# Cjen1/stateright

Measured on AMD Instinct MI355X. Metric: unique states/sec (whole node) + HBM GB/s, 2pc N=9 at 1/2/4/8 MI355X, higher is better.
Workload: dtype u64; 1 GPU; 2pc N=9 spawn_bfs, full check per step (10340352 unique states); model=2pc, rm_count=9, order=fast, parallelism=1 GPU, world_size=1

## Files before the change

include/stateright_gpu.h:

```cpp
#ifndef STATERIGHT_GPU_H
#define STATERIGHT_GPU_H

#include <stdint.h>

#ifdef __cplusplus
extern "C" {
#endif

enum sr_model_id {
    SR_MODEL_LINEAR_EQUATION = 1,
    SR_MODEL_BINARY_CLOCK = 2,
    SR_MODEL_2PC = 3,
    SR_MODEL_INCREMENT = 4,
    SR_MODEL_INCREMENT_LOCK = 5,
    SR_MODEL_DGRAPH = 6,
    SR_MODEL_PAXOS = 7,
    SR_MODEL_PINGPONG = 9,
    SR_MODEL_ACTOR_FIXTURE = 10,
    SR_MODEL_ABD = 11,
    SR_MODEL_SINGLE_COPY = 12,
    SR_MODEL_LADDER = 13,
    SR_MODEL_SPREAD = 14
};

enum sr_order {
    SR_ORDER_AUTO = 0,
    SR_ORDER_FIFO = 1,
    SR_ORDER_FAST = 2
};

enum sr_expectation { SR_ALWAYS = 0, SR_EVENTUALLY = 1, SR_SOMETIMES = 2 };

enum sr_status {
    SR_OK = 0,
    SR_ERR_ARG = -1,
    SR_ERR_HIP = -2,
    SR_ERR_CAPACITY = -3,
    SR_ERR_UNSUPPORTED = -4,
    SR_ERR_NO_DEVICE = -5,
    SR_ERR_NONDETERMINISM = -6
};

typedef struct sr_opts {
    uint32_t struct_size;
    int32_t device;
    uint64_t target_state_count;
    int32_t order;
    int32_t record_visits;
    uint64_t capacity_hint;
    int32_t profile;
    int32_t verbose;
    int32_t counters;
    int32_t defer_paths;
    int32_t symmetry;
} sr_opts;

typedef struct sr_stats {
    double level_loop_sec;
    double total_sec;
    double expand_kernel_ms;
    uint64_t expand_launches;
    uint64_t levels;
    uint64_t table_capacity;
    uint64_t rehashes;
    uint64_t algorithmic_bytes;
    uint64_t successors;
    uint32_t words_per_state;
    uint32_t order_used;
    uint32_t restarts;
    uint32_t pipelined;
    uint64_t records_routed;
    uint64_t head_levels;
    uint64_t probes;
    uint64_t cas;
    uint64_t max_displacement;
    uint32_t displacement_limit;
    uint32_t table_doublings;
    uint32_t exchange_fallbacks;
    uint32_t owner_key;
    uint32_t balanced_levels;
    uint32_t table_encoding;
} sr_stats;

typedef struct sr_bfs sr_bfs;

void sr_opts_init(sr_opts* opts);
void sr_opts_init_sized(sr_opts* opts, uint32_t size);
const char* sr_last_error(void);
int sr_device_count(void);

sr_bfs* sr_gpu_bfs_spawn(int32_t model_id, const int64_t* params, int32_t nparams, const sr_opts* opts);
int32_t sr_gpu_bfs_join(sr_bfs* bfs);
int32_t sr_gpu_bfs_is_done(const sr_bfs* bfs);
int32_t sr_gpu_bfs_is_running(const sr_bfs* bfs);
uint64_t sr_gpu_bfs_state_count(const sr_bfs* bfs);
uint64_t sr_gpu_bfs_unique_state_count(const sr_bfs* bfs);
uint32_t sr_gpu_bfs_max_depth(const sr_bfs* bfs);
int32_t sr_gpu_bfs_stats(const sr_bfs* bfs, sr_stats* out);
int32_t sr_gpu_bfs_stats_sized(const sr_bfs* bfs, sr_stats* out, uint32_t size);
int64_t sr_gpu_bfs_launch_profile(const sr_bfs* bfs, double* kernel_ms, uint64_t* frontier, int64_t cap);
int64_t sr_gpu_bfs_launch_counters(const sr_bfs* bfs, uint64_t* probes, uint64_t* cas, int64_t cap);

int32_t sr_gpu_bfs_property_count(const sr_bfs* bfs);
int32_t sr_gpu_bfs_property(const sr_bfs* bfs, int32_t prop, char* name, int32_t cap, int32_t* expectation);

int32_t sr_gpu_bfs_discovery(const sr_bfs* bfs, int32_t prop, uint64_t* fp_chain, uint32_t cap);
int32_t sr_gpu_bfs_discovery_path(const sr_bfs* bfs, int32_t prop, int64_t* action_ids, int32_t cap_actions,
                                  int64_t* states, int64_t cap_states);
int32_t sr_gpu_bfs_describe_width(const sr_bfs* bfs);
int32_t sr_gpu_bfs_action_name(const sr_bfs* bfs, int64_t action_id, char* buf, int32_t cap);
int64_t sr_gpu_bfs_action_id_bound(const sr_bfs* bfs);
int32_t sr_gpu_bfs_init_count(const sr_bfs* bfs);
int32_t sr_gpu_bfs_replay(const sr_bfs* bfs, int32_t init_index, const int64_t* action_ids, int32_t n_actions,
                          int64_t* states, int64_t cap_states, int32_t* conditions, int32_t cap_conditions);
int32_t sr_gpu_bfs_replay_trace(const sr_bfs* bfs, int32_t init_index, const int64_t* action_ids, int32_t n_actions,
                                int32_t* conditions, int64_t cap, int32_t* terminal);
int32_t sr_gpu_bfs_explore(const sr_bfs* bfs, const uint64_t* fingerprints, int32_t n, int64_t* action_ids,
                           int32_t* has_state, uint64_t* fingerprints_out, int64_t* states, int32_t cap);
int64_t sr_gpu_bfs_visits(const sr_bfs* bfs, int64_t* out, int64_t cap);
int64_t sr_gpu_bfs_visit_tree(const sr_bfs* bfs, int64_t* parent, int64_t* action, int64_t cap);
void sr_gpu_bfs_free(sr_bfs* bfs);

#define SR_DIST_ID_BYTES 128
typedef struct sr_dist sr_dist;
int32_t sr_dist_unique_id(uint8_t* id_out);
sr_dist* sr_dist_init(int32_t rank, int32_t world, const uint8_t* id, int32_t device);
int32_t sr_dist_local_group(int32_t world, const int32_t* devices, sr_dist** comms_out);
sr_dist* sr_dist_shm_init(int32_t rank, int32_t world, const char* name, int32_t device, int64_t slot_bytes,
                          int32_t devices_distinct);
int32_t sr_dist_rank(const sr_dist* comm);
int32_t sr_dist_world(const sr_dist* comm);
int32_t sr_dist_nranks(const sr_dist* comm);
int32_t sr_dist_kind(const sr_dist* comm, char* buf, int32_t cap);
int32_t sr_dist_barrier(sr_dist* comm);
int32_t sr_dist_allreduce_f64(sr_dist* comm, double* values, int32_t n, int32_t op);
void sr_dist_free(sr_dist* comm);

typedef struct sr_dist_host_opts {
    uint32_t struct_size;
    int32_t rm_count;
    uint64_t cmin;
    int32_t corrupt_level;
    int32_t capacity_fail_at_end;
    int32_t fail_at_end;
    int32_t plan_div;
} sr_dist_host_opts;
typedef struct sr_dist_host_result {
    uint64_t unique, state_count, local_unique;
    uint32_t max_depth, levels;
    uint32_t attempts, restarts, fallbacks, disagreements;
    uint32_t overflow_level;
    uint32_t first_outcome;
    uint64_t plan_digest;
} sr_dist_host_result;
int32_t sr_dist_host_protocol(const char* name, int32_t rank, int32_t world, const sr_dist_host_opts* opts,
                              sr_dist_host_result* out);

int32_t sr_rccl_version(int32_t* runtime, int32_t* compiled);
int32_t sr_hip_runtime_version(int32_t* runtime, int32_t* compiled);
int32_t sr_device_synchronize(int32_t device);
const char* sr_build_digest(void);
int32_t sr_selftest_tables(void);
int32_t sr_selftest_level_geometry(void);
int32_t sr_selftest_models(void);
int32_t sr_selftest_action_masks(void);
int32_t sr_selftest_table_growth(void);
int32_t sr_table_encoding(int32_t words, int32_t key_bits, uint64_t slots, uint32_t* out);
sr_bfs* sr_gpu_bfs_spawn_partitioned(sr_dist* comm, int32_t virtual_partitions, int32_t model_id,
                                     const int64_t* params, int32_t nparams, const sr_opts* opts);

#define SR_PLUGIN_ABI 4
typedef struct sr_plugin {
    uint32_t abi;
    uint32_t opts_size;
    const char* name;
    void* (*create)(const int64_t* params, int32_t nparams, const sr_opts* opts, void* comm, int32_t virtual_parts,
                    char* err, int32_t errcap);
    int32_t (*fingerprint)(const int64_t* params, int32_t nparams, const int64_t* described, int32_t width,
                           uint64_t* fp_out);
} sr_plugin;

sr_bfs* sr_gpu_bfs_spawn_plugin(const sr_plugin* plugin, const int64_t* params, int32_t nparams, const sr_opts* opts);
sr_bfs* sr_gpu_bfs_spawn_plugin_partitioned(const sr_plugin* plugin, sr_dist* comm, int32_t virtual_partitions,
                                            const int64_t* params, int32_t nparams, const sr_opts* opts);

int32_t sr_model_fingerprint(int32_t model_id, const int64_t* params, int32_t nparams, const int64_t* described,
                             int32_t width, uint64_t* fp_out);
int64_t sr_selftest_describe(int32_t model_id, const int64_t* params, int32_t nparams, int64_t max_states);

#ifdef __cplusplus
}
#endif
#endif
```

stateright_amd/_native.py:

```python
import ctypes
import os

HERE = os.path.dirname(os.path.abspath(__file__))
LIB_PATH = os.environ.get("SR_LIB_PATH") or os.path.join(HERE, "libstateright_gpu.so")

SR_MODEL_LINEAR_EQUATION = 1
SR_MODEL_BINARY_CLOCK = 2
SR_MODEL_2PC = 3
SR_MODEL_INCREMENT = 4
SR_MODEL_INCREMENT_LOCK = 5
SR_MODEL_DGRAPH = 6
SR_MODEL_PAXOS = 7
SR_MODEL_PINGPONG = 9
SR_MODEL_ACTOR_FIXTURE = 10
SR_MODEL_ABD = 11
SR_MODEL_SINGLE_COPY = 12
SR_MODEL_LADDER = 13
SR_MODEL_SPREAD = 14

SR_ORDER_AUTO, SR_ORDER_FIFO, SR_ORDER_FAST = 0, 1, 2
SR_ALWAYS, SR_EVENTUALLY, SR_SOMETIMES = 0, 1, 2


class sr_opts(ctypes.Structure):
    _fields_ = [
        ("struct_size", ctypes.c_uint32),
        ("device", ctypes.c_int32),
        ("target_state_count", ctypes.c_uint64),
        ("order", ctypes.c_int32),
        ("record_visits", ctypes.c_int32),
        ("capacity_hint", ctypes.c_uint64),
        ("profile", ctypes.c_int32),
        ("verbose", ctypes.c_int32),
        ("counters", ctypes.c_int32),
        ("defer_paths", ctypes.c_int32),
        ("symmetry", ctypes.c_int32),
    ]


class sr_stats(ctypes.Structure):
    _fields_ = [
        ("level_loop_sec", ctypes.c_double),
        ("total_sec", ctypes.c_double),
        ("expand_kernel_ms", ctypes.c_double),
        ("expand_launches", ctypes.c_uint64),
        ("levels", ctypes.c_uint64),
        ("table_capacity", ctypes.c_uint64),
        ("rehashes", ctypes.c_uint64),
        ("algorithmic_bytes", ctypes.c_uint64),
        ("successors", ctypes.c_uint64),
        ("words_per_state", ctypes.c_uint32),
        ("order_used", ctypes.c_uint32),
        ("restarts", ctypes.c_uint32),
        ("pipelined", ctypes.c_uint32),
        ("records_routed", ctypes.c_uint64),
        ("head_levels", ctypes.c_uint64),
        ("probes", ctypes.c_uint64),
        ("cas", ctypes.c_uint64),
        ("max_displacement", ctypes.c_uint64),
        ("displacement_limit", ctypes.c_uint32),
        ("table_doublings", ctypes.c_uint32),
        ("exchange_fallbacks", ctypes.c_uint32),
        ("owner_key", ctypes.c_uint32),
        ("balanced_levels", ctypes.c_uint32),
        ("table_encoding", ctypes.c_uint32),
    ]

    def as_dict(self):
        return {name: getattr(self, name) for name, _ in self._fields_}


class sr_dist_host_opts(ctypes.Structure):
    _fields_ = [
        ("struct_size", ctypes.c_uint32),
        ("rm_count", ctypes.c_int32),
        ("cmin", ctypes.c_uint64),
        ("corrupt_level", ctypes.c_int32),
        ("capacity_fail_at_end", ctypes.c_int32),
        ("fail_at_end", ctypes.c_int32),
        ("plan_div", ctypes.c_int32),
    ]


class sr_dist_host_result(ctypes.Structure):
    _fields_ = [
        ("unique", ctypes.c_uint64),
        ("state_count", ctypes.c_uint64),
        ("local_unique", ctypes.c_uint64),
        ("max_depth", ctypes.c_uint32),
        ("levels", ctypes.c_uint32),
        ("attempts", ctypes.c_uint32),
        ("restarts", ctypes.c_uint32),
        ("fallbacks", ctypes.c_uint32),
        ("disagreements", ctypes.c_uint32),
        ("overflow_level", ctypes.c_uint32),
        ("first_outcome", ctypes.c_uint32),
        ("plan_digest", ctypes.c_uint64),
    ]

    def as_dict(self):
        return {name: getattr(self, name) for name, _ in self._fields_}


_P = ctypes.c_void_p
_I64P = ctypes.POINTER(ctypes.c_int64)
SIGNATURES = [
    ("sr_opts_init", None, [ctypes.POINTER(sr_opts)]),
    ("sr_opts_init_sized", None, [ctypes.POINTER(sr_opts), ctypes.c_uint32]),
    ("sr_last_error", ctypes.c_char_p, []),
    ("sr_device_count", ctypes.c_int, []),
    ("sr_gpu_bfs_spawn", _P, [ctypes.c_int32, _I64P, ctypes.c_int32, ctypes.POINTER(sr_opts)]),
    ("sr_gpu_bfs_join", ctypes.c_int32, [_P]),
    ("sr_gpu_bfs_is_done", ctypes.c_int32, [_P]),
    ("sr_gpu_bfs_is_running", ctypes.c_int32, [_P]),
    ("sr_gpu_bfs_state_count", ctypes.c_uint64, [_P]),
    ("sr_gpu_bfs_unique_state_count", ctypes.c_uint64, [_P]),
    ("sr_gpu_bfs_max_depth", ctypes.c_uint32, [_P]),
    ("sr_gpu_bfs_stats", ctypes.c_int32, [_P, ctypes.POINTER(sr_stats)]),
    ("sr_gpu_bfs_stats_sized", ctypes.c_int32, [_P, ctypes.POINTER(sr_stats), ctypes.c_uint32]),
    ("sr_gpu_bfs_launch_counters", ctypes.c_int64, [_P, ctypes.POINTER(ctypes.c_uint64), ctypes.POINTER(ctypes.c_uint64),
                                                    ctypes.c_int64]),
    ("sr_gpu_bfs_launch_profile", ctypes.c_int64, [_P, ctypes.POINTER(ctypes.c_double), ctypes.POINTER(ctypes.c_uint64),
                                                   ctypes.c_int64]),
    ("sr_gpu_bfs_property_count", ctypes.c_int32, [_P]),
    ("sr_gpu_bfs_property", ctypes.c_int32, [_P, ctypes.c_int32, ctypes.c_char_p, ctypes.c_int32,
                                             ctypes.POINTER(ctypes.c_int32)]),
    ("sr_gpu_bfs_discovery", ctypes.c_int32, [_P, ctypes.c_int32, ctypes.POINTER(ctypes.c_uint64), ctypes.c_uint32]),
    ("sr_gpu_bfs_discovery_path", ctypes.c_int32, [_P, ctypes.c_int32, _I64P, ctypes.c_int32, _I64P, ctypes.c_int64]),
    ("sr_gpu_bfs_describe_width", ctypes.c_int32, [_P]),
    ("sr_gpu_bfs_action_name", ctypes.c_int32, [_P, ctypes.c_int64, ctypes.c_char_p, ctypes.c_int32]),
    ("sr_gpu_bfs_action_id_bound", ctypes.c_int64, [_P]),
    ("sr_gpu_bfs_init_count", ctypes.c_int32, [_P]),
    ("sr_gpu_bfs_replay", ctypes.c_int32, [_P, ctypes.c_int32, _I64P, ctypes.c_int32, _I64P, ctypes.c_int64,
                                           ctypes.POINTER(ctypes.c_int32), ctypes.c_int32]),
    ("sr_gpu_bfs_replay_trace", ctypes.c_int32, [_P, ctypes.c_int32, _I64P, ctypes.c_int32, ctypes.POINTER(ctypes.c_int32),
                                                 ctypes.c_int64, ctypes.POINTER(ctypes.c_int32)]),
    ("sr_gpu_bfs_explore", ctypes.c_int32, [_P, ctypes.POINTER(ctypes.c_uint64), ctypes.c_int32, _I64P,
                                            ctypes.POINTER(ctypes.c_int32), ctypes.POINTER(ctypes.c_uint64), _I64P,
                                            ctypes.c_int32]),
    ("sr_gpu_bfs_visits", ctypes.c_int64, [_P, _I64P, ctypes.c_int64]),
    ("sr_gpu_bfs_visit_tree", ctypes.c_int64, [_P, _I64P, _I64P, ctypes.c_int64]),
    ("sr_gpu_bfs_free", None, [_P]),
    ("sr_dist_unique_id", ctypes.c_int32, [ctypes.c_char_p]),
    ("sr_dist_init", _P, [ctypes.c_int32, ctypes.c_int32, ctypes.c_char_p, ctypes.c_int32]),
    ("sr_dist_local_group", ctypes.c_int32, [ctypes.c_int32, ctypes.POINTER(ctypes.c_int32), ctypes.POINTER(_P)]),
    ("sr_dist_shm_init", _P, [ctypes.c_int32, ctypes.c_int32, ctypes.c_char_p, ctypes.c_int32, ctypes.c_int64,
                              ctypes.c_int32]),
    ("sr_dist_rank", ctypes.c_int32, [_P]),
    ("sr_dist_world", ctypes.c_int32, [_P]),
    ("sr_dist_nranks", ctypes.c_int32, [_P]),
    ("sr_dist_kind", ctypes.c_int32, [_P, ctypes.c_char_p, ctypes.c_int32]),
    ("sr_dist_barrier", ctypes.c_int32, [_P]),
    ("sr_dist_allreduce_f64", ctypes.c_int32, [_P, ctypes.POINTER(ctypes.c_double), ctypes.c_int32, ctypes.c_int32]),
    ("sr_dist_free", None, [_P]),
    ("sr_dist_host_protocol", ctypes.c_int32, [ctypes.c_char_p, ctypes.c_int32, ctypes.c_int32,
                                               ctypes.POINTER(sr_dist_host_opts), ctypes.POINTER(sr_dist_host_result)]),
    ("sr_rccl_version", ctypes.c_int32, [ctypes.POINTER(ctypes.c_int32), ctypes.POINTER(ctypes.c_int32)]),
    ("sr_hip_runtime_version", ctypes.c_int32, [ctypes.POINTER(ctypes.c_int32), ctypes.POINTER(ctypes.c_int32)]),
    ("sr_device_synchronize", ctypes.c_int32, [ctypes.c_int32]),
    ("sr_build_digest", ctypes.c_char_p, []),
    ("sr_selftest_tables", ctypes.c_int32, []),
    ("sr_selftest_level_geometry", ctypes.c_int32, []),
    ("sr_selftest_models", ctypes.c_int32, []),
    ("sr_selftest_action_masks", ctypes.c_int32, []),
    ("sr_selftest_table_growth", ctypes.c_int32, []),
    ("sr_table_encoding", ctypes.c_int32, [ctypes.c_int32, ctypes.c_int32, ctypes.c_uint64, ctypes.POINTER(ctypes.c_uint32)]),
    ("sr_gpu_bfs_spawn_plugin", _P, [_P, _I64P, ctypes.c_int32, ctypes.POINTER(sr_opts)]),
    ("sr_gpu_bfs_spawn_plugin_partitioned", _P, [_P, _P, ctypes.c_int32, _I64P, ctypes.c_int32,
                                                 ctypes.POINTER(sr_opts)]),
    ("sr_model_fingerprint", ctypes.c_int32, [ctypes.c_int32, _I64P, ctypes.c_int32, _I64P, ctypes.c_int32,
                                              ctypes.POINTER(ctypes.c_uint64)]),
    ("sr_selftest_describe", ctypes.c_int64, [ctypes.c_int32, _I64P, ctypes.c_int32, ctypes.c_int64]),
    ("sr_gpu_bfs_spawn_partitioned", _P, [_P, ctypes.c_int32, ctypes.c_int32, _I64P, ctypes.c_int32,
                                          ctypes.POINTER(sr_opts)]),
]

SR_DIST_ID_BYTES = 128

_lib = None


def load():
    global _lib
    if _lib is None:
        if not os.path.exists(LIB_PATH):
            raise ImportError(
                f"MI355X engine library not found at {LIB_PATH}; build it with "
                "`python -c 'import __graft_entry__ as g; g.build()'` (hipcc --offload-arch=gfx950)")
        lib = ctypes.CDLL(LIB_PATH)
        ab = os.environ.get("SR_LIB_DIGEST_CHECK", "1") == "0"
        for name, res, args in SIGNATURES:
            fn = getattr(lib, name, None)
            if fn is None and ab:
                continue
            if fn is None:
                raise ImportError(f"{LIB_PATH} lacks {name}: rebuild it")
            fn.restype = res
            fn.argtypes = args
        check_digest(lib)
        _lib = lib
    return _lib


class StaleLibraryError(ImportError):
    pass


def check_digest(lib, sources_root=None):
    if os.environ.get("SR_LIB_DIGEST_CHECK", "1") == "0":
        return
    from . import build
    want = build.source_digest() if sources_root is None else build.source_digest_at(sources_root)
    got = lib.sr_build_digest().decode()
    if got != want:
        raise StaleLibraryError(
            f"{LIB_PATH} was built from sources with digest {got}, but the sources here have digest {want}; "
            "rebuild it (`python -c 'import __graft_entry__ as g; g.build()'`)")


def build_digest():
    lib = load()
    return lib.sr_build_digest().decode() if hasattr(lib, "sr_build_digest") else "unstamped"


def last_error():
    return load().sr_last_error().decode(errors="replace")


def table_encoding(words, key_bits, slots):
    out = (ctypes.c_uint32 * 8)()
    st = load().sr_table_encoding(words, key_bits, slots, out)
    if st != 0:
        raise ValueError(f"sr_table_encoding: {last_error()} (status {st})")
    return dict(zip(("qbits", "dbits", "bbits", "plimit", "s32", "filter", "filter_log2", "min_cap_log2"), out))


def runtime_versions():
    lib = load()
    out = {}
    for key, fn in (("hip", lib.sr_hip_runtime_version), ("rccl", lib.sr_rccl_version)):
        r, c = ctypes.c_int32(), ctypes.c_int32()
        out[key] = (r.value, c.value) if fn(ctypes.byref(r), ctypes.byref(c)) == 0 else (None, None)
    return out


def loaded_runtime_paths():
    paths = set()
    try:
        with open("/proc/self/maps") as f:
            for line in f:
                p = line.split()[-1] if line.count(" ") >= 5 else ""
                if "libamdhip64" in p or "librccl" in p:
                    paths.add(p)
    except OSError:
        pass
    return sorted(paths)
```

stateright_amd/csrc/device.hpp:

```cpp
#pragma once
#include <hip/hip_runtime.h>

#include <chrono>
#include <cstdint>
#include <cstdio>
#include <cstdlib>
#include <cstring>
#include <map>
#include <mutex>
#include <stdexcept>
#include <string>
#include <tuple>
#include <vector>

namespace sr {

struct Error : std::runtime_error {
    int code;
    Error(int c, const std::string& m) : std::runtime_error(m), code(c) {}
};

#define SR_HIP(expr)                                                                              \
    do {                                                                                          \
        hipError_t e_ = (expr);                                                                   \
        if (e_ != hipSuccess)                                                                     \
            throw ::sr::Error(-2, std::string(#expr) + ": " + hipGetErrorString(e_) + " at " +   \
                                      __FILE__ + ":" + std::to_string(__LINE__));                 \
    } while (0)

inline void clear_not_ready() {
    if (hipPeekAtLastError() == hipErrorNotReady) (void)hipGetLastError();
}
inline hipError_t stream_sync(hipStream_t s) {
    const auto t0 = std::chrono::steady_clock::now();
    for (unsigned spin = 1;; ++spin) {
        const hipError_t e = hipStreamQuery(s);
        if (e != hipErrorNotReady) {
            if (spin > 1) clear_not_ready();
            return e;
        }
        if ((spin & 255) == 0 && std::chrono::steady_clock::now() - t0 > std::chrono::microseconds(500))
            return clear_not_ready(), hipStreamSynchronize(s);
        __builtin_ia32_pause();
    }
}

struct StreamCensus {
    static StreamCensus& get() {
        static StreamCensus c;
        return c;
    }
    void created(int dev) {
        std::lock_guard<std::mutex> g(mu_);
        ++n_[dev];
    }
    void destroyed(int dev) {
        std::lock_guard<std::mutex> g(mu_);
        --n_[dev];
    }
    int on(int dev) {
        std::lock_guard<std::mutex> g(mu_);
        return n_[dev];
    }
    static int hw_queues() {
        const char* e = std::getenv("GPU_MAX_HW_QUEUES");
        return e && std::atoi(e) > 0 ? std::atoi(e) : 4;
    }
    std::mutex mu_;
    std::map<int, int> n_;
};
inline hipError_t create_stream(hipStream_t* s, int dev) {
    const hipError_t e = hipStreamCreateWithFlags(s, hipStreamNonBlocking);
    if (e == hipSuccess) StreamCensus::get().created(dev);
    return e;
}

class DevicePool {
  public:
    static DevicePool& get() {
        static DevicePool p;
        return p;
    }
    void* alloc(int dev, size_t bytes, int kind = 0) {
        bytes = round(bytes);
        {
            std::lock_guard<std::mutex> g(mu_);
            auto& fl = free_[{dev, bytes, kind}];
            if (!fl.empty()) {
                void* p = fl.back();
                fl.pop_back();
                return p;
            }
            if (kind == 0)
                if (void* p = take_zeroed_locked(dev, bytes)) return p;
        }
        void* p = nullptr;
        auto raw = [&]() {
            return kind == 1   ? hipExtMallocWithFlags(&p, bytes, hipDeviceMallocFinegrained)
                   : kind == 2 ? hipExtMallocWithFlags(&p, bytes, hipDeviceMallocUncached)
                               : hipMalloc(&p, bytes);
        };
        const auto t0 = std::chrono::steady_clock::now();
        hipError_t e = raw();
        const bool retried = e != hipSuccess;
        if (retried) {
            release_all(dev);
            (void)hipGetLastError();
            SR_HIP(raw());
        }
        if (trace())
            std::fprintf(stderr, "[pool] device %d: %zu bytes (kind %d) fresh%s in %.3f ms\n", dev, bytes, kind,
                         retried ? " after emptying the cache" : "",
                         std::chrono::duration<double, std::milli>(std::chrono::steady_clock::now() - t0).count());
        return p;
    }
    void free(int dev, void* p, size_t bytes, int kind = 0) {
        if (!p) return;
        std::lock_guard<std::mutex> g(mu_);
        free_[{dev, round(bytes), kind}].push_back(p);
    }
    void free_zeroed(int dev, void* p, size_t bytes, hipEvent_t ready, int kind = 0) {
        std::lock_guard<std::mutex> g(mu_);
        zeroed_[{dev, round(bytes), kind}].push_back({p, ready});
    }
    void* alloc_zeroed(int dev, size_t bytes, hipStream_t s, int kind = 0) {
        Zeroed z{nullptr, nullptr};
        {
            std::lock_guard<std::mutex> g(mu_);
            auto& fl = zeroed_[{dev, round(bytes), kind}];
            if (fl.empty()) return nullptr;
            size_t pick = 0;
            for (size_t i = 0; i < fl.size(); ++i)
                if (hipEventQuery(fl[i].ready) == hipSuccess) {
                    pick = i;
                    break;
                }
            clear_not_ready();
            z = fl[pick];
            fl.erase(fl.begin() + (long)pick);
        }
        const hipError_t e = hipStreamWaitEvent(s, z.ready, 0);
        if (e != hipSuccess) {
            (void)hipEventSynchronize(z.ready);
            (void)hipEventDestroy(z.ready);
            free(dev, z.p, bytes, kind);
            return nullptr;
        }
        (void)hipEventDestroy(z.ready);
        return z.p;
    }
    void release_all(int dev) {
        std::lock_guard<std::mutex> g(mu_);
        ++epoch_[dev];
        for (auto& [k, v] : free_)
            if (std::get<0>(k) == dev) {
                for (void* p : v) (void)hipFree(p);
                v.clear();
            }
        for (auto& [k, v] : zeroed_)
            if (std::get<0>(k) == dev) {
                for (auto& z : v) {
                    (void)hipEventSynchronize(z.ready);
                    (void)hipEventDestroy(z.ready);
                    (void)hipFree(z.p);
                }
                v.clear();
            }
    }
    static bool trace() {
        static const bool on = std::getenv("SR_POOL_TRACE") && std::atoi(std::getenv("SR_POOL_TRACE")) != 0;
        return on;
    }
    static size_t round(size_t b) {
        if (b < 256) return 256;
        if (b >= (2u << 20)) return (b + (2u << 20) - 1) & ~(size_t)((2u << 20) - 1);
        size_t r = 256;
        while (r < b) r <<= 1;
        return r;
    }

    uint64_t epoch(int dev) {
        std::lock_guard<std::mutex> g(mu_);
        return epoch_[dev];
    }

  private:
    struct Zeroed {
        void* p;
        hipEvent_t ready;
    };
    void* take_zeroed_locked(int dev, size_t bytes) {
        auto it = zeroed_.find({dev, bytes, 0});
        if (it == zeroed_.end()) return nullptr;
        auto& fl = it->second;
        for (size_t i = 0; i < fl.size(); ++i) {
            if (hipEventQuery(fl[i].ready) != hipSuccess) continue;
            Zeroed z = fl[i];
            fl.erase(fl.begin() + (long)i);
            (void)hipEventDestroy(z.ready);
            clear_not_ready();
            return z.p;
        }
        clear_not_ready();
        return nullptr;
    }
    std::mutex mu_;
    std::map<std::tuple<int, size_t, int>, std::vector<void*>> free_;
    std::map<std::tuple<int, size_t, int>, std::vector<Zeroed>> zeroed_;
    std::map<int, uint64_t> epoch_;
};

template <class T>
struct DBuf {
    T* p = nullptr;
    size_t n = 0;
    int dev = 0;
    int kind = 0;
    DBuf() = default;
    DBuf(const DBuf&) = delete;
    DBuf& operator=(const DBuf&) = delete;
    DBuf(DBuf&& o) noexcept { swap(o); }
    ~DBuf() { reset(); }
    void reset() {
        if (p) DevicePool::get().free(dev, p, n * sizeof(T), kind);
        p = nullptr;
        n = 0;
        kind = 0;
    }
    void alloc(int d, size_t count, int k = 0) {
        reset();
        dev = d;
        n = count ? count : 1;
        kind = k;
        p = static_cast<T*>(DevicePool::get().alloc(d, n * sizeof(T), k));
    }
    void alloc_zero(int d, size_t count, hipStream_t s, int k = 0) {
        reset();
        dev = d;
        n = count ? count : 1;
        kind = k;
        p = static_cast<T*>(DevicePool::get().alloc_zeroed(d, n * sizeof(T), s, k));
        if (p) return;
        p = static_cast<T*>(DevicePool::get().alloc(d, n * sizeof(T), k));
        SR_HIP(hipMemsetAsync(p, 0, n * sizeof(T), s));
    }
    void release_zero(hipStream_t s) noexcept {
        if (!p) return;
        hipEvent_t ready = nullptr;
        if (hipEventCreateWithFlags(&ready, hipEventDisableTiming) == hipSuccess) {
            if (hipMemsetAsync(p, 0, n * sizeof(T), s) == hipSuccess && hipEventRecord(ready, s) == hipSuccess) {
                DevicePool::get().free_zeroed(dev, p, n * sizeof(T), ready, kind);
                p = nullptr;
                n = 0;
                kind = 0;
                return;
            }
            (void)hipEventDestroy(ready);
        }
        (void)hipStreamSynchronize(s);
        (void)hipGetLastError();
        reset();
    }
    void swap(DBuf& o) {
        std::swap(p, o.p);
        std::swap(n, o.n);
        std::swap(dev, o.dev);
        std::swap(kind, o.kind);
    }
};

template <class Counters, class HostMirror>
struct DeviceContext {
    int dev = 0;
    hipStream_t stream = nullptr;
    Counters* lc = nullptr;
    HostMirror* hc = nullptr;
    HostMirror* hc_dev = nullptr;
    uint32_t seq = 0;
    std::vector<hipEvent_t> events;
    hipEvent_t done = nullptr;

    void init(int d) {
        dev = d;
        SR_HIP(hipSetDevice(d));
        SR_HIP(create_stream(&stream, d));
        SR_HIP(hipEventCreateWithFlags(&done, hipEventDisableTiming));
        SR_HIP(hipMalloc(&lc, sizeof(Counters)));
        SR_HIP(hipHostMalloc(&hc, 2 * sizeof(HostMirror), hipHostMallocCoherent | hipHostMallocMapped));
        SR_HIP(hipHostGetDevicePointer(reinterpret_cast<void**>(&hc_dev), hc, 0));
        std::memset(hc, 0, 2 * sizeof(HostMirror));
    }
    hipEvent_t event(size_t i) {
        while (events.size() <= i) {
            hipEvent_t e;
            SR_HIP(hipEventCreate(&e));
            events.push_back(e);
        }
        return events[i];
    }
};

template <class Ctx>
class ContextPool {
  public:
    static ContextPool& get() {
        static ContextPool p;
        return p;
    }
    Ctx* acquire(int dev) {
        {
            std::lock_guard<std::mutex> g(mu_);
            auto& fl = free_[dev];
            if (!fl.empty()) {
                Ctx* c = fl.back();
                fl.pop_back();
                return c;
            }
        }
        auto* c = new Ctx();
        c->init(dev);
        return c;
    }
    void release(Ctx* c) {
        if (!c) return;
        std::lock_guard<std::mutex> g(mu_);
        free_[c->dev].push_back(c);
    }

  private:
    std::mutex mu_;
    std::map<int, std::vector<Ctx*>> free_;
};

}
// ... 1 lines not shown
```

stateright_amd/csrc/engine.hip:

```cpp
#include <unordered_set>
#include "registry.hpp"
#include "dgraph.hpp"
#include "paxos.hpp"
#include "abd_wide.hpp"
#include "dist_host.hpp"
#include "table_selftest.hpp"

namespace sr {

static thread_local std::string g_last_error;
static void set_error(const std::string& e) { g_last_error = e; }

}

namespace sr {

static std::unique_ptr<EngineBase> make_model_engine(const EngineArgs& a) {
    if (a.o->symmetry && a.model != SR_MODEL_2PC)
        throw Error(SR_ERR_UNSUPPORTED, "symmetry reduction: model " + std::to_string(a.model) + " has no canonical form");
    switch (a.model) {
        case SR_MODEL_LINEAR_EQUATION:
        case SR_MODEL_BINARY_CLOCK:
        case SR_MODEL_DGRAPH:
        case SR_MODEL_ACTOR_FIXTURE:
// ... 812 lines not shown
int32_t sr_hip_runtime_version(int32_t* runtime, int32_t* compiled) {
    int v = 0;
    if (hipRuntimeGetVersion(&v) != hipSuccess) return SR_ERR_HIP;
    if (runtime) *runtime = v;
    if (compiled) *compiled = HIP_VERSION;
    return SR_OK;
}

int32_t sr_selftest_tables(void) {
    for (u32 B = 1; B <= 18; ++B) {
        std::vector<u8> seen(1u << B, 0);
        for (u64 x = 0; x < (1ull << B); ++x) {
            const u64 y = (u64)qperm(x, B);
            if (y >> B || seen[y]) {
                set_error("qperm is not a bijection on " + std::to_string(B) + " bits");
                return SR_ERR_ARG;
            }
            seen[y] = 1;
        }
    }
    for (u32 B = 2; B <= 20; ++B) {
        std::vector<u8> seen(1u << B, 0);
        for (u64 x = 0; x < (1ull << B); ++x) {
            const u64 y = qmix(x, B);
            if (y >> B || seen[y]) {
                set_error("qmix is not a bijection on " + std::to_string(B) + " bits");
                return SR_ERR_ARG;
            }
            seen[y] = 1;
        }
    }
    const u32 ncases[][2] = {{40, 25}, {40, 22}, {44, 27}, {48, 29}, {52, 31}, {16, 22}, {62, 40}};
    u64 rn = 0x452821E638D01377ull;
    for (auto& c : ncases) {
        const u32 q = c[0] > c[1] ? c[0] - c[1] : 1u;
        TableView t{nullptr, nullptr, (1ull << c[1]) - 1, q, 32 - q, c[0]};
        t.s32 = 1;
        if (q + SLOT32_DMIN > 32) {
            t.s32 = 0;
            t.dbits = 64 - q;
        }
        for (int i = 0; i < 100000; ++i) {
            rn = fmix64(rn + 0x9E3779B97F4A7C15ull);
            const u64 key = rn & ((1ull << c[0]) - 1);
            const u64 h = qmix(key, c[0]);
            const ProbeKey pk = quot_probe(t, h);
            const u64 d = (rn >> 40) % 500;
            const u64 slotv = pk.tag + d;
            if ((t.s32 && slotv >> 32) || quot_decode(t, (pk.home + d) & t.mask, slotv) != h || pk.home > t.mask ||
                filter_key(t, pk) != h + 1) {
                set_error("narrow quotient slot encode/decode mismatch at B=" + std::to_string(c[0]));
                return SR_ERR_ARG;
            }
        }
    }
    const u32 cases[][2] = {{89, 33}, {68, 20}, {82, 26}, {120, 64}};
    u64 r = 0x243F6A8885A308D3ull;
    for (auto& c : cases) {
        TableView t{nullptr, nullptr, (c[1] >= 64 ? ~0ull : (1ull << c[1]) - 1), c[0] - c[1], 64 - (c[0] - c[1]), c[0]};
        for (int i = 0; i < 100000; ++i) {
            r = fmix64(r + 0x9E3779B97F4A7C15ull);
            const u64 r2 = fmix64(r ^ 0xABCDEFull);
            const u128 key = ((u128)r2 << 64 | r) & (((u128)1 << c[0]) - 1);
            const u128 h = qperm(key, c[0]);
            const ProbeKey pk = quot_probe(t, h);
            const u64 d = r2 % 200;
            if (quot_decode(t, (pk.home + d) & t.mask, pk.tag + d) != h || pk.home > t.mask || (pk.tag & ((1ull << t.dbits) - 1)) != 1) {
                set_error("quotient slot encode/decode mismatch at B=" + std::to_string(c[0]));
                return SR_ERR_ARG;
            }
        }
    }
    return SR_OK;
}

int32_t sr_selftest_table_growth(void) {
    try {
        std::string why;
        if (!table_growth_selftest(why)) {
            set_error(why);
            return SR_ERR_ARG;
        }
        return SR_OK;
    } catch (const std::exception& x) {
        set_error(x.what());
        return SR_ERR_ARG;
    }
}

int32_t sr_table_encoding(int32_t words, int32_t key_bits, uint64_t slots, uint32_t* out) {
    try {
        if (!out || key_bits < 2 || (words != 1 && words != 2 && words != 4) || key_bits > std::min(64 * words, 128) ||
            !slots || (slots & (slots - 1)))
            throw Error(SR_ERR_ARG, "sr_table_encoding: words 1, 2 or 4, 2 <= key_bits <= min(64 words, 128), slots a power of two");
        const TableEncoding e = words == 1   ? table_encoding_of<1>(key_bits, slots)
                                : words == 2 ? table_encoding_of<2>(key_bits, slots)
                                             : table_encoding_of<4>(key_bits, slots);
        const u32 v[8] = {e.qbits, e.dbits, e.bbits, e.plimit, e.s32, e.filter, e.filter_log2, e.min_cap_log2};
        std::copy(v, v + 8, out);
        return SR_OK;
    } catch (const Error& x) {
        set_error(x.what());
        return x.code;
    } catch (const std::exception& x) {
        set_error(x.what());
        return SR_ERR_ARG;
    }
}

static bool check_level_geometry(u32 nblk, std::vector<u32>& stamp, std::vector<u32>& end, u32& gen,
                                 const std::vector<u32>& ns, std::string& why) {
    for (u32 wpb : {4u, 8u})
        for (u32 cap_log2 = 2; cap_log2 <= 6; ++cap_log2)
            for (int balanced = 0; balanced < 2; ++balanced)
                for (u32 n : ns) {
                    const u32 cap = 1u << cap_log2, lo = n & 1 ? 77u : 0u, hi = lo + n;
                    const LevelGeom g = level_geometry(n, nblk, wpb, cap, balanced != 0);
                    auto fail = [&](const char* what) {
                        why = std::string("level geometry: ") + what + " at n=" + std::to_string(n) + " nblk=" +
                              std::to_string(nblk) + " cap=" + std::to_string(cap) + " wpb=" + std::to_string(wpb) +
                              (balanced ? " balanced" : " fixed");
                        return false;
                    };
                    if (g.pw == 0 || g.pw > cap || g.cw == 0 || g.cw > wpb * cap) return fail("pw or cw out of range");
                    if (!balanced && (g.pw != cap || g.cw != wpb * cap)) return fail("fixed geometry changed");
                    ++gen;
                    u64 intervals = 0, share_min = ~0ull, share_max = 0;
                    for (u32 b = 0; b < nblk; ++b) {
                        u64 share = 0;
                        u64 j = 0;
                        for (u64 c0 = g.first_chunk(lo, b); c0 < hi; c0 += g.stride(nblk), ++j) {
                            const u32 lim = g.chunk_end(c0, hi);
                            for (u32 wid = 0; wid < wpb; ++wid) {
                                const u64 w0 = g.wave_first(c0, wid);
                                const u64 w1 = std::min<u64>(w0 + g.pw, lim);
                                if (!balanced) {
                                    const u64 o0 = lo + (((u64)b + j * nblk) * wpb << cap_log2) + ((u64)wid << cap_log2);
                                    const u64 o1 = std::min<u64>(o0 + cap, hi);
                                    if (o0 < o1 ? o0 != w0 || o1 != w1 : w0 < w1) return fail("differs from the shift formula");
                                }
                                if (w1 <= w0) continue;
                                if (w0 < lo || w1 > hi) return fail("a parent outside the frontier");
                                if (stamp[w0 - lo] == gen) return fail("a parent taken twice");
                                stamp[w0 - lo] = gen;
                                end[w0 - lo] = (u32)(w1 - lo);
                                share += w1 - w0;
                                ++intervals;
                            }
                        }
                        share_min = std::min(share_min, share);
                        share_max = std::max(share_max, share);
                    }
                    u64 followed = 0;
                    u32 pos = 0;
                    while (pos < n) {
                        if (stamp[pos] != gen) return fail("a parent not taken");
                        pos = end[pos];
                        ++followed;
                    }
                    if (pos != n || followed != intervals) return fail("waves overlap");
                    if (share_max - share_min > g.cw) return fail("workgroup shares differ by more than one chunk");
                }
    return true;
}

int32_t sr_selftest_level_geometry(void) {
// ... 167 lines not shown
```

stateright_amd/csrc/engine.hpp:

```cpp
#pragma once
#include <algorithm>
#include <atomic>
#include <chrono>
#include <cmath>
#include <cstdio>
#include <cstdlib>
#include <cstring>
#include <deque>
#include <immintrin.h>
#include <memory>
#include <string>
#include <thread>
#include <vector>

#include "../../include/stateright_gpu.h"
#include "device.hpp"
#include "kernels.hpp"

namespace sr {


using Clock = std::chrono::steady_clock;
static double secs(Clock::time_point a, Clock::time_point b) { return std::chrono::duration<double>(b - a).count(); }

// ... 179 lines not shown
        cur.clear();
        for (int i = 0; i < k && cur.empty(); ++i) {
            u64 c[W];
            m.base().canonical(&inits[i * W], c);
            if (std::equal(c, c + W, st.begin())) cur.assign(&inits[i * W], &inits[i * W] + W);
        }
        if (cur.empty()) throw Error(SR_ERR_NONDETERMINISM, "Unable to reconstruct a `Path`: no init state has the expected representative");
    }
    auto emit = [&](const u64* s) {
        const size_t o = states.size();
        states.resize(o + wd);
        m.describe(s, &states[o]);
        if (raw) raw->insert(raw->end(), s, s + W);
    };
    for (size_t i = 1; i < len; ++i) {
        const u64* target = &st[i * W];
        u64 mask[M::MW];
        m.enabled(cur.data(), mask);
        bool found = false;
        for (int w = 0; w < M::MW && !found; ++w)
            for (u64 bits = mask[w]; bits && !found; bits &= bits - 1) {
                const int a = w * 64 + __builtin_ctzll(bits);
                u64 ns[W];
                if (!m.apply(cur.data(), a, ns) || !std::equal(ns, ns + W, target)) continue;
                u64 next[W];
                if constexpr (is_canon<M>::value) m.base().apply(cur.data(), a, next);
                else std::copy(ns, ns + W, next);
                emit(cur.data());
                actions.push_back(m.action_id(cur.data(), a));
                cur.assign(next, next + W);
                found = true;
            }
        if (!found)
            throw Error(SR_ERR_NONDETERMINISM, "Unable to reconstruct a `Path`: " + std::to_string(i) +
                                                   " previous state(s) reconstructed but no successor is the next state");
    }
    emit(cur.data());
    return (int)actions.size();
}

template <class M>
int fingerprint_chain(const M& m, const std::vector<u64>& st, std::vector<u64>& out) {
    constexpr int W = M::W;
    out.clear();
    std::vector<u64> raw;
    if constexpr (is_canon<M>::value) {
        std::vector<i64> actions, described;
        concrete_path(m, st, actions, described, &raw);
    } else {
        raw = st;
    }
    for (size_t i = 0; i < raw.size() / W; ++i) out.push_back(state_fp<M>(&raw[i * W]));
    return (int)out.size();
}

template <class M>
class Engine final : public EngineBase {
    static constexpr int W = M::W;
    static constexpr u32 WPB = (u32)expand_wpb<M>();

  public:
    Engine(M m, const sr_opts& o)
        : m_(m), o_(o), A_((u32)m.max_actions()), D_((u32)m.max_out_degree()), emask_(model_emask(m)) {
        disc.resize(M::NPROPS);
        (void)init_states_of(m_);
        if (const char* e = std::getenv("SR_PROBE_BATCH")) probe_batch_ = std::atoi(e);
        if (const char* e = std::getenv("SR_TABLE_LOAD")) table_load_ = std::atof(e), load_env_ = true;
        if (const char* e = std::getenv("SR_PPW_LOG2")) ppw_env_ = std::atoi(e);
        if (const char* e = std::getenv("SR_FILTER_LOG2")) filt_log2_ = (u32)std::atoi(e);
        if (!filter_exact(m_)) filt_log2_ = 0;
        if (filt_log2_ && (!std::getenv("SR_FILTER_COMPACT") || std::atoi(std::getenv("SR_FILTER_COMPACT"))) &&
            filter_compact_ok(m_, filt_log2_ + 1))
            filt_log2_ += 1, filt_compact_ = true;
        grid_res_ = W == 1 ? 1u : 2u;
        if (const char* e = std::getenv("SR_GRID_RES"))
            if (std::atoi(e) > 0) grid_res_ = (u32)std::atoi(e);
        if (const char* e = std::getenv("SR_PIPELINE")) pipeline_ = std::atoi(e) != 0;
        if (const char* e = std::getenv("SR_QUERY_LOG2")) query_mask_ = (1ull << std::atoi(e)) - 1;
        if (const char* e = std::getenv("SR_GRID_MAX")) grid_env_ = (u32)std::max(0, std::atoi(e));
        if (const char* e = std::getenv("SR_WIDE_NOPF")) wide_nopf_ = std::atoi(e) ? 1 : 0;
        if (const char* e = std::getenv("SR_CHAIN_MAX")) chain_max_ = (u64)std::max(0ll, std::atoll(e));
        if (const char* e = std::getenv("SR_TABLE_KIND")) table_kind_ = std::atoi(e);
        if (const char* e = std::getenv("SR_TABLE_RECYCLE")) table_recycle_ = std::atoi(e) != 0;
        if (const char* e = std::getenv("SR_BALANCE")) balance_ = std::atoi(e) != 0;
        if (const char* e = std::getenv("SR_BALANCE_MIN")) balance_min_ = (u64)std::max(0ll, std::atoll(e));
        action_table_ = action_table_model<M> && A_ <= 64;
        if (const char* e = std::getenv("SR_ACTION_TABLE")) action_table_ = action_table_ && std::atoi(e) != 0;
    }
    ~Engine() override = default;

    int nprops() const override { return M::NPROPS; }
    const char* prop_name(int p) const override { return m_.prop_name(p); }
    int expectation(int p) const override { return m_.expectation(p); }
    int width() const override { return m_.describe_width(); }
    std::string action_name(i64 id) const override { return m_.action_name(id); }

    void run() override {
        SR_HIP(hipSetDevice(o_.device));
        CtxLease lease(o_.device);
        bind(lease.c);
        int order = o_.order;
        if (order == SR_ORDER_AUTO) order = o_.target_state_count ? SR_ORDER_FIFO : SR_ORDER_FAST;
        if (emask_ && o_.order != SR_ORDER_FAST) order = SR_ORDER_FIFO;
        bool order_dependent = run_with_restart(order);
        if (order_dependent && o_.order == SR_ORDER_AUTO && order == SR_ORDER_FAST) {
            if (o_.verbose) std::fprintf(stderr, "[sr] early exit in FAST order; re-running in FIFO order\n");
            run_with_restart(SR_ORDER_FIFO);
        }
        bind(nullptr);
    }

    bool run_with_restart(int order) {
        for (int attempt = 0;; ++attempt) {
            try {
                return run_order(order);
            } catch (const Error& e) {
                if (e.code != SR_ERR_CAPACITY || attempt >= 3) throw;
                if (o_.verbose) std::fprintf(stderr, "[sr] %s; restarting with larger buffers\n", e.what());
                pessimistic_ = true;
                grow_factor_ *= 4;
                (void)stream_sync(stream_);
                rehash_pending_ = false;
                retired_keys_.clear();
                retired_arena_.clear();
                retired_u32_.clear();
                init_counters();
            }
        }
    }

    int chain(int p, std::vector<u64>& out) override {
        out.clear();
        if (p < 0 || p >= M::NPROPS || !disc[p].found) return 0;
        SR_HIP(hipSetDevice(o_.device));
        std::vector<u64> st;
        tree_path(disc[p].level, disc[p].rank, st);
        return fingerprint_chain(m_, st, out);
    }

    void tree_path(u32 level, u32 rank, std::vector<u64>& st) {
        std::vector<u64> idx;
        u64 r = rank;
        for (int d = (int)level;; --d) {
            u64 a = lstart_[d] + r;
            idx.push_back(a);
            if (d == 0) break;
            u32 pr = 0;
            SR_HIP(hipMemcpy(&pr, apar_.p + a, sizeof(u32), hipMemcpyDeviceToHost));
            r = pr;
        }
        std::reverse(idx.begin(), idx.end());
        st.resize(idx.size() * W);
        for (size_t i = 0; i < idx.size(); ++i)
            SR_HIP(hipMemcpy(&st[i * W], arena_.p + idx[i] * W, W * sizeof(u64), hipMemcpyDeviceToHost));
    }

    int path(int p, std::vector<i64>& actions, std::vector<i64>& states) override {
        if (p < 0 || p >= M::NPROPS || !disc[p].found) return -1;
        SR_HIP(hipSetDevice(o_.device));
        std::vector<u64> st;
        tree_path(disc[p].level, disc[p].rank, st);
        return concrete_path(m_, st, actions, states);
    }

    i64 action_id_bound() const override { return m_.action_id_bound(); }
    int init_count() const override { return (int)(init_states_of(base_model(m_)).size() / std::decay_t<decltype(base_model(m_))>::W); }
    int replay(int init, const i64* ids, int n, std::vector<i64>& states, std::vector<int>& conds,
               std::vector<int>* all_conds, int* terminal) const override {
        return replay_model(base_model(m_), init, ids, n, states, conds, all_conds, terminal);
    }
    int explore(const u64* fps, int n, std::vector<i64>& action, std::vector<int>& has, std::vector<u64>& fp,
                std::vector<i64>& states) const override {
        return explore_model(base_model(m_), fps, n, action, has, fp, states);
    }

    bool visit_tree(std::vector<i64>& parent, std::vector<i64>& action) const override {
        parent.clear();
        action.clear();
        std::vector<u64> prev_states;
        i64 prev_base = 0;
        for (size_t d = 0; d < lvisited_.size(); ++d) {
            const u64 nv = lvisited_[d];
            std::vector<u64> st(nv * W);
            std::vector<u32> par(nv);
            if (nv) {
                SR_HIP(hipMemcpy(st.data(), arena_.p + lstart_[d] * W, nv * W * sizeof(u64), hipMemcpyDeviceToHost));
                SR_HIP(hipMemcpy(par.data(), apar_.p + lstart_[d], nv * sizeof(u32), hipMemcpyDeviceToHost));
            }
            const i64 base = (i64)parent.size();
            for (u64 i = 0; i < nv; ++i) {
                if (d == 0) {
                    parent.push_back(-1);
                    action.push_back(-1);
                    continue;
                }
                const u64 pr = par[i];
                if (pr >= prev_states.size() / W) throw Error(SR_ERR_NONDETERMINISM, "visit parent outside the visited prefix");
                const u64* ps = &prev_states[pr * W];
                const u64 want = state_fp<M>(&st[i * W]);
                u64 mask[M::MW];
                m_.enabled(ps, mask);
                i64 id = -1;
                for (int w = 0; w < M::MW && id < 0; ++w)
                    for (u64 bits = mask[w]; bits && id < 0; bits &= bits - 1) {
                        const int a = w * 64 + __builtin_ctzll(bits);
                        u64 ns[W];
                        if (m_.apply(ps, a, ns) && state_fp<M>(ns) == want) id = m_.action_id(ps, a);
                    }
                if (id < 0) throw Error(SR_ERR_NONDETERMINISM, "Unable to reconstruct a `Path` for a visited state");
                parent.push_back(prev_base + (i64)pr);
                action.push_back(id);
            }
            prev_states.swap(st);
            prev_base = base;
        }
        return true;
    }

    std::vector<i64> visits() const override {
        const int wd = m_.describe_width();
        std::vector<u64> st;
        for (size_t d = 0; d < lvisited_.size(); ++d) {
            size_t o = st.size();
            st.resize(o + lvisited_[d] * W);
            if (lvisited_[d])
                SR_HIP(hipMemcpy(&st[o], arena_.p + lstart_[d] * W, lvisited_[d] * W * sizeof(u64), hipMemcpyDeviceToHost));
        }
        std::vector<i64> out(st.size() / W * wd);
        for (size_t i = 0; i < st.size() / W; ++i) m_.describe(&st[i * W], &out[i * wd]);
        return out;
    }

  private:
    TableView view() const { return make_table_view(m_, keys_.p, fifo_ ? meta_.p : nullptr, cap_); }

    void alloc_table(u64 cap, bool zero = true) {
        cap_ = cap;
        lmax_ = max_load(cap);
        const u64 words = table_words(make_table_view(m_, nullptr, nullptr, cap), cap);
        table_unzeroed_ = false;
        if (zero) keys_.alloc_zero(o_.device, words, stream_, table_kind_);
        else keys_.alloc(o_.device, words, table_kind_);
        if (fifo_) {
            meta_.alloc(o_.device, cap);
            SR_HIP(hipMemsetAsync(meta_.p, 0xff, cap * sizeof(u64), stream_));
        }
    }

    void grow_table(u32* cand = nullptr, u64 cand_n = 0, u64 min_slots = 0) {
        check_async_growth();
        const auto tg = Clock::now();
        DBuf<u64> ok, om;
        ok.swap(keys_);
        if (fifo_) om.swap(meta_);
        const TableView from = make_table_view(m_, ok.p, fifo_ ? om.p : nullptr, cap_);
        const u64 old_cap = cap_;
        if (!aux_.p) aux_.alloc(o_.device, 2);
        u64 f0 = 2;
        while (old_cap * f0 < min_slots) f0 *= 2;
        for (u64 f = f0;; f *= 2) {
            launch_rehash(from, old_cap, f);
            u32 err = 0;
            SR_HIP(hipMemcpyAsync(&err, aux_.p, sizeof(u32), hipMemcpyDeviceToHost, stream_));
            SR_HIP(stream_sync(stream_));
            if (!err) break;
            if (f >= 64) throw Error(SR_ERR_CAPACITY, "rehash: probe limit exceeded at 64x the capacity");
        }
        if (cand && cand_n) {
            remap_slots<<<blocks_for(cand_n, 256), 256, 0, stream_>>>(cand, cand_n, from, view());
            SR_HIP(hipGetLastError());
        }
        SR_HIP(stream_sync(stream_));
        stats.rehashes++;
        if (o_.verbose)
            std::fprintf(stderr, "[sr] visited set %llu -> %llu slots in %.3f ms\n", (unsigned long long)old_cap,
                         (unsigned long long)cap_, secs(tg, Clock::now()) * 1e3);
    }

    void grow_table_async(u64 min_slots) {
        check_async_growth_pending_first();
        retired_keys_.emplace_back();
        retired_keys_.back().swap(keys_);
        const TableView from = make_table_view(m_, retired_keys_.back().p, nullptr, cap_);
        const u64 old_cap = cap_;
        if (!aux_.p) aux_.alloc(o_.device, 2);
        u64 f = 2;
        while (old_cap * f < min_slots) f *= 2;
        launch_rehash(from, old_cap, f);
        rehash_pending_ = true;
        stats.rehashes++;
        if (o_.verbose)
            std::fprintf(stderr, "[sr] visited set %llu -> %llu slots enqueued\n", (unsigned long long)old_cap,
                         (unsigned long long)cap_);
    }
    void launch_rehash(const TableView& from, u64 old_cap, u64 f) {
        const u64 cap = old_cap * f;
        const TableView to0 = make_table_view(m_, nullptr, nullptr, cap);
        u32 lg = 0;
        while ((1ull << lg) < f) ++lg;
        const u64 S = to0.s32 ? rebuild_slots<u32>() : rebuild_slots<u64>();
        const bool ranges = rehash_ranges_ && !from.meta && rehash_by_ranges(from, to0, lg, cap);
        alloc_table(cap, !ranges);
        table_unzeroed_ = ranges;
        SR_HIP(hipMemsetAsync(aux_.p, 0, sizeof(u32), stream_));
        if (ranges) {
            const u64 nranges = cap / S, spill_cap = nranges + 65536;
            if (spill_.n < spill_cap + 1) spill_.alloc(o_.device, spill_cap + 1);
            SR_HIP(hipMemsetAsync(spill_.p, 0, sizeof(u64), stream_));
            if (to0.s32)
                rehash_ranges<u32><<<(u32)nranges, REBUILD_BLOCK, 0, stream_>>>(from, old_cap, view(), lg, spill_.p,
                                                                               spill_cap, aux_.p);
            else
                rehash_ranges<u64><<<(u32)nranges, REBUILD_BLOCK, 0, stream_>>>(from, old_cap, view(), lg, spill_.p,
                                                                               spill_cap, aux_.p);
            SR_HIP(hipGetLastError());
            rehash_spill<<<256, 256, 0, stream_>>>(from, view(), spill_.p, spill_cap, aux_.p);
        } else {
            rehash<<<blocks_for(old_cap, 256), 256, 0, stream_>>>(from, old_cap, view(), aux_.p);
        }
        SR_HIP(hipGetLastError());
    }
    bool rehash_ranges_ = !std::getenv("SR_REHASH_RANGES") || std::atoi(std::getenv("SR_REHASH_RANGES")) != 0;
    DBuf<u64> spill_;
    bool table_unzeroed_ = false;

    void check_async_growth_pending_first() {
        if (rehash_pending_) check_async_growth();
    }
    void check_async_growth() {
        if (!rehash_pending_ && retired_keys_.empty() && retired_arena_.empty()) return;
        SR_HIP(stream_sync(stream_));
        retired_keys_.clear();
        retired_arena_.clear();
        retired_u32_.clear();
        if (!rehash_pending_) return;
        rehash_pending_ = false;
        u32 err = 0;
        SR_HIP(hipMemcpy(&err, aux_.p, sizeof(u32), hipMemcpyDeviceToHost));
        if (err) throw Error(SR_ERR_CAPACITY, "an enqueued rehash exceeded the new table's probe limit");
    }
    bool rehash_pending_ = false;
    std::vector<DBuf<u64>> retired_keys_, retired_arena_;
    std::vector<DBuf<u32>> retired_u32_;

    u64 growth_slots(u64 need_slots) const {
        const u64 step = !o_.capacity_hint && stats.rehashes == 0 && grow_first_ ? grow_first_ : grow_step_;
        u64 target = std::max<u64>(need_slots, cap_ * step);
        size_t free_b = 0, total_b = 0;
        if (hipMemGetInfo(&free_b, &total_b) == hipSuccess && free_b) target = std::min<u64>(target, std::max<u64>(need_slots, free_b / 4 / 8));
        return target;
    }
    u64 grow_step_ = std::getenv("SR_GROW_STEP") && std::atoi(std::getenv("SR_GROW_STEP")) >= 2
                         ? (u64)std::atoi(std::getenv("SR_GROW_STEP")) : 8u;
    u64 grow_first_ = std::getenv("SR_GROW_FIRST") ? (u64)std::atoi(std::getenv("SR_GROW_FIRST")) : 0u;

    double max_load(u64 cap) const {
        const TableView v = make_table_view(m_, nullptr, nullptr, cap, true);
        return max_load_for(v.plimit, (double)cap, 0.8);
    }

    void displacement_stats() {
        const TableView v = view();
        stats.displacement_limit = v.plimit;
        stats.table_encoding = table_encoding_word(v, filt_log2_, filt_compact_);
        if (!o_.counters || !cap_) return;
        if (!aux_.p) aux_.alloc(o_.device, 2);
        SR_HIP(hipMemsetAsync(aux_.p + 1, 0, sizeof(u32), stream_));
        const u32 grid = (u32)std::min<u64>(blocks_for(cap_, 256), 8192);
        table_max_disp<<<grid, 256, 0, stream_>>>(v, cap_, aux_.p + 1);
        SR_HIP(hipGetLastError());
        u32 d = 0;
        SR_HIP(hipMemcpyAsync(&d, aux_.p + 1, sizeof(u32), hipMemcpyDeviceToHost, stream_));
        SR_HIP(stream_sync(stream_));
        stats.max_displacement = d;
    }

    u64 arena_step_ = std::getenv("SR_ARENA_STEP") && std::atoi(std::getenv("SR_ARENA_STEP")) >= 2
                          ? (u64)std::atoi(std::getenv("SR_ARENA_STEP")) : W <= 2 ? 8u : 4u;
    void ensure_arena(u64 states, u64 used, bool async = false) {
        if (arena_cap_ >= states) return;
        const auto ta = Clock::now();
        u64 cap = std::max<u64>(states, arena_cap_ * (arena_cap_ ? arena_step_ : 1));
        if (cap > states) {
            size_t fr = 0, tot = 0;
            const u64 per = W * sizeof(u64) + sizeof(u32) + (emask_ ? sizeof(u32) : 0);
            if (hipMemGetInfo(&fr, &tot) == hipSuccess) cap = std::max<u64>(states, std::min<u64>(cap, fr / 2 / per));
            else (void)hipGetLastError();
        }
        DBuf<u64> na;
        DBuf<u32> np, ne;
        na.alloc(o_.device, cap * W);
        np.alloc(o_.device, cap);
        if (emask_) ne.alloc(o_.device, cap);
        const double alloc_ms = secs(ta, Clock::now()) * 1e3;
        if (used) {
            SR_HIP(hipMemcpyAsync(na.p, arena_.p, used * W * sizeof(u64), hipMemcpyDeviceToDevice, stream_));
            SR_HIP(hipMemcpyAsync(np.p, apar_.p, used * sizeof(u32), hipMemcpyDeviceToDevice, stream_));
            if (emask_) SR_HIP(hipMemcpyAsync(ne.p, aeb_.p, used * sizeof(u32), hipMemcpyDeviceToDevice, stream_));
        }
        const bool had = arena_.p != nullptr;
        arena_.swap(na);
        apar_.swap(np);
        if (emask_) aeb_.swap(ne);
        arena_cap_ = cap;
        if (had && async) {
            retired_arena_.emplace_back();
            retired_arena_.back().swap(na);
            retired_u32_.emplace_back();
            retired_u32_.back().swap(np);
            retired_u32_.emplace_back();
            retired_u32_.back().swap(ne);
        } else if (had) {
            SR_HIP(stream_sync(stream_));
        }
        if (o_.verbose && had)
            std::fprintf(stderr, "[sr] arena -> %llu states (%llu copied) in %.3f ms (allocation %.3f ms)\n",
                         (unsigned long long)cap, (unsigned long long)used, secs(ta, Clock::now()) * 1e3, alloc_ms);
    }

    void bind(Ctx* c) {
        ctx_ = c;
        stream_ = c ? c->stream : nullptr;
        lc_d_ = c ? c->lc : nullptr;
    }

    void init_counters() {
        if (!slots_.p) slots_.alloc(o_.device, (SLOTS * sizeof(LevelCounters) + 7) / 8);
        init_level_counters<<<1, 256, 0, stream_>>>(lc_d_, reinterpret_cast<LevelCounters*>(slots_.p), SLOTS);
        SR_HIP(hipGetLastError());
        slot_k_ = 0;
        slot_published_ = true;
    }

    LevelCounters* slot(u32 k) const { return reinterpret_cast<LevelCounters*>(slots_.p) + (k % SLOTS); }
    SlotWork slot_work(bool dev_n) {
        SlotWork sw{};
        if (dev_n) sw.prev_n = slot_k_ ? &slot(slot_k_ - 1)->claims : &lc_d_->prev_claims;
        if (slot_k_ && !slot_published_) {
            sw.pub = slot(slot_k_ - 1);
            sw.hc = hcd(slot_seq_);
            sw.seq = slot_seq_;
            slot_published_ = true;
        }
        if (slot_k_ >= 2) sw.zero = slot(slot_k_ - 2);
        return sw;
    }
    void publish_pending_slot() {
// ... 351 lines not shown
        };
        u32 sq = sq_level0;
        std::deque<u32> ahead;
        vt0_ = Clock::now();
        for (;;) {
            const double g = std::max(ratio_, 1.0) * 1.5;
            const u64 est1 = (u64)((double)n * g) + 1024;
            const u64 est2 = (u64)((double)est1 * g) + 1024;
            const u64 est3 = (u64)((double)est2 * g) + 1024;
            const u64 nb_next = lstart_.back();
            const u64 shape = (u64)((double)n * std::max(ratio_, 0.05) * 1.1) + 64;
            if (ahead.empty() && !pessimistic_ && !o_.capacity_hint && n <= early_grow_max_ &&
                (double)(unique + est1 + est2 + est3) >= lmax_ * (double)cap_) {
                const u64 want = unique + est1 + est2 + est3;
                grow_table_async(growth_slots((u64)((double)want / lmax_) + 1));
                if (nb_next + est1 + est2 + est3 > arena_cap_) ensure_arena(nb_next + est1 + est2 + est3, arena_cap_, true);
                if (o_.verbose) std::fprintf(stderr, "[sr] early growth at a frontier of %llu states\n", (unsigned long long)n);
            }
            if (ahead.empty()) {
                const bool spec = !pessimistic_ && (double)(unique + est1 + est2) < lmax_ * (double)cap_ &&
                                  nb_next + est1 + est2 <= arena_cap_;
                if (spec) ahead.push_back(launch_expand(nb_next, 0, true, shape, undiscovered));
            }
            if (ahead.size() == 1 && chain_max_ && est1 <= chain_max_ && !pessimistic_ &&
                (double)(unique + est1 + est2 + est3) < lmax_ * (double)cap_ && nb_next + est1 + est2 + est3 <= arena_cap_) {
                const u64 shape2 = (u64)((double)shape * std::max(ratio_, 0.05) * 1.1) + 64;
                ahead.push_back(launch_expand(0, 0, true, shape2, undiscovered, 0, true));
            }
            if (ahead.empty()) publish_pending_slot();

            bool spec_ok = !ahead.empty();
            if (!wait_publish(sq, true)) {
                if (lc_.err == ERR_DEFERRED) {
                    SR_HIP(stream_sync(stream_));
                    init_counters();
                    if (o_.verbose)
                        std::fprintf(stderr, "[sr] level of %llu states outgrew the room planned for it: deferred\n",
                                     (unsigned long long)n);
                    const u32 s2 = launch_sync(n, undiscovered);
                    publish_pending_slot();
                    if (!wait_publish(s2, true)) repair_level(lstart_[lstart_.size() - 2], n, undiscovered);
                } else {
                    repair_level(lstart_[lstart_.size() - 2], n, undiscovered);
                }
                spec_ok = false;
            }
            auto it = seq_launch_.find(sq);
            if (it != seq_launch_.end() && it->second < launch_frontier.size()) {
                launch_frontier[it->second] = n;
                launch_probes[it->second] = lc_.probes;
                launch_cas[it->second] = lc_.cas;
            }
            if (!spec_ok) ahead.clear();
            if (!account(lc_, ahead.size() == 2 ? " (next two enqueued)" : spec_ok ? " (next enqueued)" : "")) break;
            if (!ahead.empty()) {
                sq = ahead.front();
                ahead.pop_front();
            } else {
                sq = launch_sync(n, undiscovered);
            }
        }
        SR_HIP(hipEventRecord(ctx_->done, stream_));
        release_table();
        drain(ctx_->done);
        check_async_growth();
        free_unzeroed_table();
        return order_dependent;
    }

    void drain(hipEvent_t ev = nullptr) {
        if (!ev) {
            SR_HIP(stream_sync(stream_));
            return;
        }
        for (;;) {
            const hipError_t e = hipEventQuery(ev);
            if (e == hipSuccess) return clear_not_ready();
            if (e != hipErrorNotReady) SR_HIP(e);
            _mm_pause();
        }
    }

    void release_table() {
        if (table_recycle_ && !fifo_ && !o_.counters && !table_unzeroed_) keys_.release_zero(stream_);
    }
    void free_unzeroed_table() {
        if (!table_recycle_ || fifo_ || o_.counters || !table_unzeroed_ || !keys_.p) return;
        SR_HIP(stream_sync(stream_));
        keys_.reset();
    }

    u32 launch_sync(u64 n, u32 undiscovered) {
        const u64 d_eff = pessimistic_ ? D_ : std::min<u64>(D_, (u64)std::ceil(2.0 * recent_ratio() + 1.0));
        const double need = (double)(unique + n * d_eff);
        const u64 fbase = lstart_[lstart_.size() - 2];
        if (need > lmax_ * (double)cap_) {
            grow_table(nullptr, 0, growth_slots((u64)(need / lmax_) + 1));
            if ((double)arena_cap_ < lmax_ * (double)cap_) ensure_arena(arena_cap_ + 1, fbase + n);
        }
        ensure_arena(fbase + n + n * d_eff, fbase + n);
        return launch_expand(fbase, (u32)n, false, n, undiscovered);
    }

    u32 expand_grid_cap(bool nopf = false, bool deep = false) {
        const int form = (nopf ? 2 : probe_loop() < 0 ? 1 : 0) + (deep && !nopf ? 3 : 0);
        u32& cap = grid_max_[form];
        if (cap) return cap;
        if (grid_env_) return cap = grid_env_;
        int per_cu = 0, cus = 0;
        const size_t dyn = filt_bytes();
        const void* k = form == 1 ? (const void*)expand_fast<M, -4, 0> : (const void*)expand_fast<M, 1, 0>;
        if (form == 3) k = (const void*)expand_fast<M, 1, 0, false, false, true>;
        if (form == 4) k = (const void*)expand_fast<M, -4, 0, false, false, true>;
        if constexpr (W >= 4)
            if (nopf) k = (const void*)expand_fast<M, 1, 0, false, true>;
        SR_HIP(hipOccupancyMaxActiveBlocksPerMultiprocessor(&per_cu, k, 64 * WPB, dyn));
        SR_HIP(hipDeviceGetAttribute(&cus, hipDeviceAttributeMultiprocessorCount, o_.device));
        cap = per_cu > 0 && cus > 0 ? (u32)(grid_res_ * per_cu * cus) : ~0u;
        if (o_.verbose)
            std::fprintf(stderr, "[sr] expand grid cap %u blocks (%d per CU x %d CUs x %u)%s\n", cap, per_cu, cus, grid_res_,
                         nopf ? " [no prefetch]" : form >= 3 ? " [dynamic chunks]" : "");
        return cap;
    }
    bool balance_level(u64 shape, bool dev_n, bool deep) {
        if (!balance_ || deep || (dev_n ? shape < balance_min_ : balance_min_ == ~0ull)) return false;
        stats.balanced_levels++;
        return true;
    }
    template <class L>
    void launch_form(L& launch, bool nopf, bool deep, bool bal) {
        if (o_.counters) bal ? launch(expand_fast<M, 1, 0, true, false, false, true>) : launch(expand_fast<M, 1, 0, true>);
        else if (nopf) launch_nopf(launch, bal);
        else if (deep) probe_loop() < 0 ? launch(expand_fast<M, -4, 0, false, false, true>) : launch(expand_fast<M, 1, 0, false, false, true>);
        else if (probe_loop() < 0) bal ? launch(expand_fast<M, -4, 0, false, false, false, true>) : launch(expand_fast<M, -4, 0>);
        else bal ? launch(expand_fast<M, 1, 0, false, false, false, true>) : launch(expand_fast<M, 1, 0>);
    }
    bool action_table_ = false;
    bool balance_ = true;
    u64 balance_min_ = W == 1 ? (u64)1 << 16 : ~0ull;
    bool deep_level(u64 chunks, u32 grid) const {
        return SR_DYN_CHUNKS && W < 4 && dyn_env_ && grid >= DYN_SHARDS && chunks > (u64)DYN_MIN_RATIO * grid;
    }
    bool dyn_env_ = !std::getenv("SR_DYN") || std::atoi(std::getenv("SR_DYN")) != 0;
    bool use_nopf(u64 chunks) {
        if constexpr (W < 4) return false;
        if (o_.counters || wide_nopf_ == 0) return false;
        if (wide_nopf_ == 1) return true;
        return chunks <= expand_grid_cap(true);
    }

    u32 launch_expand(u64 fbase, u32 n, bool dev_n, u64 shape, u32 undiscovered, u32 flags = 0, bool chained = false) {
        const u32 sq = next_seq();
        if (chained) fbase = 0;
        const u64 nbase = fbase + (dev_n ? 0 : n);
        const u32 ncap = (u32)std::min<u64>(arena_cap_ - nbase, 0xffffffffu);
        const u32 ppw_log2 = ppw_env_ >= 0 ? (u32)ppw_env_ : ppw_for(shape);
        const u32 chunks = std::max<u32>(1, blocks_for((shape + (1u << ppw_log2) - 1) >> ppw_log2, WPB));
        const bool nopf = use_nopf(chunks);
        u32 grid = std::min(expand_grid_cap(nopf), chunks);
        const bool deep = !o_.counters && !nopf && deep_level(chunks, grid);
        if (deep) grid = std::min(expand_grid_cap(false, true), chunks);
        const bool bal = balance_level(shape, dev_n, deep);
        seq_launch_[sq] = launch_frontier.size();
        SlotWork sw = slot_work(dev_n);
        sw.flags = flags | (action_table_ ? (u32)SLOT_ACTION_TABLE : 0u);
        sw.arena = arena_.p;
        sw.apar = apar_.p;
// ... 97 lines not shown
            };
            if (!wait_publish(launch_chunk(false), true)) {
                const HostCounters first = lc_;
                u32 dmin[MAX_PROPS];
                std::copy(first.disc, first.disc + MAX_PROPS, dmin);
                for (int attempt = 0;; ++attempt) {
                    if (attempt >= 8) throw Error(SR_ERR_CAPACITY, "visited set probe limit exceeded after 8 doublings");
                    grow_table(fifo_ ? cand.p : nullptr, fifo_ ? limit * A : 0);
                    stats.table_doublings++;
                    SR_HIP(hipMemsetD32Async(reinterpret_cast<hipDeviceptr_t>(&lc_d_->claims), (int)lc_.claims, 1, stream_));
                    SR_HIP(hipMemsetD32Async(reinterpret_cast<hipDeviceptr_t>(&lc_d_->err), 0, 1, stream_));
                    const bool ok = wait_publish(launch_chunk(true), true);
                    for (int p = 0; p < MAX_PROPS; ++p) dmin[p] = std::min(dmin[p], lc_.disc[p]);
                    if (ok) break;
                }
                lc_.successors = std::max(lc_.successors, first.successors);
                lc_.enabled = std::max(lc_.enabled, first.enabled);
                std::copy(dmin, dmin + MAX_PROPS, lc_.disc);
            }
            claims = lc_.claims;
            lo += c;
        }
        ratio_ = (double)claims / (double)limit;
        if (!fifo_) {
            en_ratio_ = std::max(1.0, (double)lc_.enabled / (double)limit);
            return claims;
        }

        ensure_arena(nbase + claims, nbase);
        DBuf<u32> counts, offs, sums, total;
        counts.alloc(o_.device, limit);
        offs.alloc(o_.device, limit);
        u32 tiles = blocks_for(limit, SCAN_TILE);
        sums.alloc(o_.device, tiles);
        total.alloc(o_.device, 1);
        timed([&] { own_count<M><<<blocks_for(limit, 256), 256, 0, stream_>>>(cand.p, (u32)limit, A, level, view(), counts.p); });
        scan_tile_sums<<<tiles, SCAN_BLOCK, 0, stream_>>>(counts.p, (u32)limit, sums.p);
        scan_sums<<<1, SCAN_BLOCK, 0, stream_>>>(sums.p, tiles, total.p);
        scan_tiles<<<tiles, SCAN_BLOCK, 0, stream_>>>(counts.p, (u32)limit, sums.p, offs.p);
        SR_HIP(hipGetLastError());
        const u32 sq = next_seq();
        timed([&] {
            scatter_fifo<M><<<blocks_for(limit, 256), 256, 0, stream_>>>(m_, cur(), cand.p, offs.p, (u32)limit, A, level,
                                                                         view(), arena_.p + nbase * W, apar_.p + nbase, lc_d_,
                                                                         undiscovered, hcd(sq), sq, total.p, peb,
                                                                         emask_ ? aeb_.p + nbase : nullptr);
        });
        wait_publish(sq);
        const u32 owners = lc_.aux;
        if (owners != claims) throw Error(SR_ERR_CAPACITY, "FIFO ownership mismatch: owners " + std::to_string(owners) + " claims " + std::to_string(claims));
        return owners;
    }

    u32 ppw_for(u64 c) const {
        const double rounds = W >= 4 ? 4.0 : 16.0;
        const double ppw = 64.0 * rounds / en_ratio_;
        const u32 lmax = expand_ppw_log2_max<M>();
        u32 l = 2;
        while (l < lmax && (double)(2u << l) <= ppw) ++l;
        while (l > 2 && ((c + (1u << l) - 1) >> l) < ppw_waves_) --l;
        return l;
    }
    u64 ppw_waves_ = std::getenv("SR_PPW_WAVES") && std::atoll(std::getenv("SR_PPW_WAVES")) > 0
                         ? (u64)std::atoll(std::getenv("SR_PPW_WAVES")) : 2048;

    const u64* cur() const { return arena_.p + lstart_[lstart_.size() - 2] * W; }

    M m_;
    sr_opts o_;
    u32 A_;
    u32 D_;
    u32 emask_;
    bool fifo_ = false;
    int probe_batch_ = 0;
    int probe_loop() const {
        if (probe_batch_) return probe_batch_ < 0 ? -4 : 1;
        constexpr bool queue_ok = W == 1 || !has_qkey<M>::value;
        if (queue_ok && W < 4 && queue_ratio_ > 0 && ratio_ >= queue_ratio_) return -4;
        return queue_ok && W < 4 && cap_ >= (1ull << 27) ? -4 : 1;
    }
    double queue_ratio_ = std::getenv("SR_QUEUE_RATIO") ? std::atof(std::getenv("SR_QUEUE_RATIO")) : 0.0;
    int ppw_env_ = -1;
    bool table_recycle_ = true;
    u32 grid_res_ = 2;
    u32 grid_max_[5] = {0, 0, 0, 0, 0};
    u32 grid_env_ = 0;
    int wide_nopf_ = -1;
    u64 chain_max_ = 16384;
    u64 early_grow_max_ = std::getenv("SR_EARLY_GROW_MAX") ? std::strtoull(std::getenv("SR_EARLY_GROW_MAX"), nullptr, 10)
                                                           : (u64)1 << 17;
    int table_kind_ = 0;
    template <class L>
    void launch_nopf(L& launch, bool bal) {
        if constexpr (W >= 4) bal ? launch(expand_fast<M, 1, 0, false, true, false, true>) : launch(expand_fast<M, 1, 0, false, true>);
    }
    u64 query_mask_ = 4095;
    bool pipeline_ = true;
    DBuf<u64> slots_;
    u32 slot_k_ = 0;
    u32 slot_seq_ = 0;
    bool slot_published_ = true;
    std::map<u32, size_t> seq_launch_;
    u32 filt_log2_ = default_filter_log2<W>();
    bool filt_compact_ = false;
    size_t filt_bytes() const { return filt_log2_ ? (size_t)(filt_compact_ ? 4u : 8u) << filt_log2_ : 0u; }
    u32 filt_arg() const { return filt_log2_ | (filt_compact_ ? FILT_COMPACT : 0u); }
    bool pessimistic_ = false;
    u64 grow_factor_ = 1;
    double ratio_ = 1.0;
    double ratios_[4] = {};
    u32 nratio_ = 0;
    void note_ratio(double r) { ratios_[nratio_++ & 3] = r; }
    double recent_ratio() const {
        double m = ratio_;
        for (u32 i = 0; i < std::min<u32>(nratio_, 4); ++i) m = std::max(m, ratios_[i]);
        return m;
    }
    double en_ratio_ = 8.0;
    double table_load_ = 0.3;
    bool load_env_ = false;
    Ctx* ctx_ = nullptr;
    hipStream_t stream_ = nullptr;
    HostCounters lc_{};
    LevelCounters* lc_d_ = nullptr;
    u64 cap_ = 0;
    DBuf<u64> keys_, meta_;
    double lmax_ = 0.8;
    Clock::time_point vt0_{};
    DBuf<u32> aux_;
    DBuf<u64> arena_;
    DBuf<u32> apar_;
    DBuf<u32> aeb_;
    u64 arena_cap_ = 0;
    std::vector<u64> lstart_;
    std::vector<u64> lvisited_;
};

}

#include "dist.hpp"

namespace sr {

template <class M>
int described_fingerprint(const M& m, const i64* d, int width, u64* fp, std::string* why = nullptr) {
    if constexpr (has_undescribe<M>::value) {
        if (!d || !fp || width != m.describe_width()) {
            if (why) *why = "bad description width";
            return SR_ERR_ARG;
        }
        u64 s[M::W];
        m.undescribe(d, s);
        std::vector<i64> back((size_t)width);
        m.describe(s, back.data());
        for (int i = 0; i < width; ++i)
            if (back[i] != d[i]) {
                if (why)
                    *why = "not a canonical state description (element " + std::to_string(i) + ": " + std::to_string(d[i]) +
                           " describes back as " + std::to_string(back[i]) + ")";
                return SR_ERR_ARG;
            }
        *fp = state_fp<M>(s);
        return SR_OK;
    } else {
        (void)m, (void)d, (void)width, (void)fp;
        if (why) *why = "model has no state description inverse";
// ... 54 lines not shown
```

stateright_amd/csrc/kernels.hpp:

```cpp
#pragma once
#include <algorithm>
#include <cmath>
#include <cstddef>
#include <cstdlib>

#include "../../include/stateright_gpu.h"
#include "device.hpp"
#include "models.hpp"

namespace sr {

constexpr u64 META_UNSET = ~0ull;
constexpr int META_SHIFT = 44;
constexpr u32 CAND_NONE = 0xffffffffu;
constexpr int MAX_PROBE = 1 << 16;
constexpr int MAX_PROPS = 32;
constexpr int MAX_PARTS = 64;
#ifndef SR_WIDE_PPW_LOG2_MAX
#define SR_WIDE_PPW_LOG2_MAX 5
#endif
#ifndef SR_STAGE_WORDS
#define SR_STAGE_WORDS 1024
#endif
#ifndef SR_DYN_CHUNKS
#define SR_DYN_CHUNKS 1
#endif
constexpr u32 DYN_SHARDS = 8;
#ifndef DYN_MIN_RATIO
#define DYN_MIN_RATIO 6
#endif
#ifndef SR_NARROW_WPB
#define SR_NARROW_WPB 4
#endif
template <class M>
constexpr int expand_wpb() { return M::W >= 4 ? 4 : SR_NARROW_WPB; }
template <class M>
constexpr u32 expand_ppw_log2_max() { return M::W >= 4 ? SR_WIDE_PPW_LOG2_MAX : expand_wpb<M>() >= 8 ? 5 : 6; }
#ifndef SR_WIDE_STAGE_WORDS
#define SR_WIDE_STAGE_WORDS 2048
#endif
#ifndef SR_WIDE_WAVES
#define SR_WIDE_WAVES 3
#endif

enum ErrBits { ERR_TABLE_FULL = 1, ERR_FRONTIER_OVERFLOW = 2, ERR_PEER_TIMEOUT = 4, ERR_EXCHANGE = 8, ERR_DEFERRED = 16,
               ERR_MODEL = 32 };

struct TableView {
    u64* keys;
    u64* meta;
    u64 mask;
    u32 qbits = 0;
    u32 dbits = 0;
    u32 bbits = 0;
    u32 plimit = MAX_PROBE;
    u32 s32 = 0;
};

template <int POL, class T>
__device__ __forceinline__ T probe_load(const T* p);
template <int POL = 0>
__device__ __forceinline__ u64 slot_load(const TableView& t, u64 i) {
    if (t.s32) return (u64)probe_load<POL>(reinterpret_cast<const u32*>(t.keys) + i);
    return probe_load<POL>(t.keys + i);
}
__device__ __forceinline__ u64 slot_cas(const TableView& t, u64 i, u64 tag) {
    if (t.s32) return (u64)atomicCAS(reinterpret_cast<u32*>(t.keys) + i, 0u, (u32)tag);
    return atomicCAS(reinterpret_cast<unsigned long long*>(t.keys + i), 0ull, (unsigned long long)tag);
}
SR_HD u64 table_words(const TableView& t, u64 cap) { return t.s32 ? (cap + 1) / 2 : cap; }

SR_HD u32 encoding_probe_limit(u32 qbits, u32 dbits) {
    return qbits && dbits < 17 ? (1u << dbits) - 2 : (u32)MAX_PROBE;
}

inline double expected_max_displacement(double alpha, double slots) {
    if (alpha <= 0) return 0;
    if (alpha >= 1) return 1e300;
    return std::log(std::max(2.0, slots)) / (alpha - 1.0 - std::log(alpha));
}
inline double max_load_for(u32 plimit, double slots, double cap_load) {
    if (plimit >= (u32)MAX_PROBE) return cap_load;
    double lo = 0.0, hi = cap_load;
    if (expected_max_displacement(hi, slots) <= plimit / 2.0) return hi;
    for (int i = 0; i < 60; ++i) {
        const double mid = 0.5 * (lo + hi);
        (expected_max_displacement(mid, slots) <= plimit / 2.0 ? lo : hi) = mid;
    }
    return lo;
}

struct ProbeKey {
    u64 home;
    u64 tag;
};

using u128 = unsigned __int128;

SR_HD u128 qperm(u128 x, u32 B) {
    const u32 hb = B / 2, ab = B - hb;
    const u64 mb = hb >= 64 ? ~0ull : (1ull << hb) - 1, ma = ab >= 64 ? ~0ull : (1ull << ab) - 1;
    u64 b = (u64)x & mb, a = (u64)(x >> hb) & ma;
    b ^= fmix64(a * 0x9E3779B97F4A7C15ull + 0x2545F4914F6CDD1Dull) & mb;
    a ^= fmix64(b * 0xC2B2AE3D27D4EB4Full + 0x165667B19E3779F9ull) & ma;
    b ^= fmix64(a * 0xD6E8FEB86659FD93ull + 0x94D049BB133111EBull) & mb;
    a ^= fmix64(b * 0xBF58476D1CE4E5B9ull + 0x7F4A7C159E3779B9ull) & ma;
    return ((u128)a << hb) | b;
}

SR_HD u64 qmix(u64 x, u32 B) {
    const u64 m = (1ull << B) - 1;
    const u32 r = (B + 1) / 2;
    x ^= x >> r;
    x = (x * 0xff51afd7ed558ccdull) & m;
    x ^= x >> r;
    x = (x * 0xc4ceb9fe1a85ec53ull) & m;
    x ^= x >> r;
    return x;
}

SR_HD u64 probe_step(const TableView& t) { return t.qbits ? 1ull : 0ull; }
SR_HD ProbeKey fp_probe(const TableView& t, u64 fp) { return ProbeKey{fp & t.mask, fp}; }
SR_HD ProbeKey quot_probe(const TableView& t, u128 h) {
    return ProbeKey{(u64)(h >> t.qbits), (((u64)h & ((1ull << t.qbits) - 1)) << t.dbits) | 1ull};
}
SR_HD u128 quot_decode(const TableView& t, u64 i, u64 v) {
    const u64 d = (v & ((1ull << t.dbits) - 1)) - 1;
    return ((u128)((i - d) & t.mask) << t.qbits) | (v >> t.dbits);
}
SR_HD ProbeKey reprobe(const TableView& from, const TableView& to, u64 i, u64 v) {
    return from.qbits ? quot_probe(to, quot_decode(from, i, v)) : fp_probe(to, v);
}

inline u32 forced_probe_limit() {
    const char* e = std::getenv("SR_DISP_LIMIT");
    return e ? (u32)std::max(1, std::atoi(e)) : 0u;
}
constexpr u32 SLOT32_DMIN = 10;
inline bool slot32_enabled() {
    static const bool on = !std::getenv("SR_SLOT32") || std::atoi(std::getenv("SR_SLOT32")) != 0;
    return on;
}
constexpr u32 QUOT_MAX_REMAINDER = 56;
template <class M>
inline bool quotient_model(const M& m) {
    if constexpr (has_qkey<M>::value) {
        const int B = m.qkey_bits();
        if constexpr (M::W == 1) return B >= 2 && B <= 62;
        else return B >= 2 && B <= 96;
    }
    (void)m;
    return false;
}
template <class M>
inline TableView make_table_view(const M& m, u64* keys, u64* meta, u64 cap, bool natural = false) {
    TableView v{keys, meta, cap - 1};
    if constexpr (has_qkey<M>::value) {
        const u32 B = (u32)m.qkey_bits();
        u32 k = 0;
        while ((1ull << k) < cap) ++k;
        if (quotient_model(m)) {
            v.qbits = B > k ? B - k : 1u;
            v.bbits = B;
            if (v.qbits > QUOT_MAX_REMAINDER)
                throw Error(SR_ERR_ARG, "make_table_view: a quotient table below min_table_cap");
            if (M::W == 1 && slot32_enabled() && v.qbits + SLOT32_DMIN <= 32) {
                v.s32 = 1;
                v.dbits = 32 - v.qbits;
            } else {
                v.dbits = 64 - v.qbits;
            }
        }
    }
    v.plimit = encoding_probe_limit(v.qbits, v.dbits);
    if (!natural && forced_probe_limit()) v.plimit = std::min(v.plimit, forced_probe_limit());
    return v;
}
template <class M>
inline u64 min_table_cap(const M& m) {
    if constexpr (has_qkey<M>::value) {
        const int B = m.qkey_bits();
        if (quotient_model(m) && B > (int)QUOT_MAX_REMAINDER) return 1ull << (B - (int)QUOT_MAX_REMAINDER);
    }
    (void)m;
    return 1;
}

template <class M>
SR_HD u128 quot_hash(const M& m, const TableView& t, const u64* s) {
    if constexpr (M::W == 1) return qmix((u64)m.qkey(s), t.bbits);
    else return qperm(m.qkey(s), t.bbits);
}

template <class M>
SR_HD ProbeKey probe_key(const M& m, const TableView& t, const u64* s) {
    if constexpr (has_qkey<M>::value) {
        if (t.qbits) return quot_probe(t, quot_hash(m, t, s));
    }
    return fp_probe(t, state_fp<M>(s));
}

SR_HD u64 filter_key(const TableView& t, const ProbeKey& k) {
    return t.qbits ? ((k.home << t.qbits) | (k.tag >> t.dbits)) + 1 : k.tag;
}
SR_HD u32 filter_index(const TableView& t, u64 fk) { return t.qbits ? (u32)fk : (u32)(fk >> 40); }
template <class M>
inline bool filter_exact(const M& m) {
    return !quotient_model(m) || M::W == 1;
}
constexpr u32 FILT_COMPACT = 0x100;
template <int W>
constexpr u32 default_filter_log2() { return W >= 4 ? 10 : 9; }
template <class M>
inline bool filter_compact_ok(const M& m, u32 log2_entries) {
    if (M::W != 1 || !filter_exact(m)) return false;
    const TableView v = make_table_view(m, nullptr, nullptr, min_table_cap(m), true);
    return v.qbits && v.bbits <= 30 + log2_entries;
}
inline u32 table_encoding_word(const TableView& t, u32 filt_log2, bool compact) {
    return t.qbits | (t.s32 ? 1u << 8 : 0u) | filt_log2 << 16 | (compact ? 1u << 24 : 0u);
}
__device__ __forceinline__ bool filter_seen(u64* filt, bool compact, u32 flog, u32 fmask, const TableView& t, u64 fk) {
    if (compact) {
        const u32 e = (u32)(fk >> flog) | 0x80000000u;
        return atomicExch(reinterpret_cast<u32*>(filt) + ((u32)fk & fmask), e) == e;
    }
    return atomicExch(reinterpret_cast<unsigned long long*>(&filt[filter_index(t, fk) & fmask]), (unsigned long long)fk) ==
           (unsigned long long)fk;
}

constexpr u32 NO_PARENT = 0xffffffffu;

struct LevelGeom {
    u32 cw, pw;
    SR_HD u64 first_chunk(u32 lo, u32 b) const { return lo + (u64)b * cw; }
    SR_HD u64 stride(u32 nblk) const { return (u64)nblk * cw; }
    SR_HD u64 wave_first(u64 c0, u32 wid) const { return c0 + (u64)wid * pw; }
    SR_HD u32 chunk_end(u64 c0, u32 hi) const { return c0 + cw < (u64)hi ? (u32)(c0 + cw) : hi; }
};
SR_HD LevelGeom level_geometry(u32 n, u32 nblk, u32 wpb, u32 cap, bool balanced) {
    if (!balanced || n == 0) return LevelGeom{wpb * cap, cap};
    const u32 per = nblk * wpb * cap;
    const u32 r = (n - 1) / per + 1;
    const u32 cw = (n - 1) / (nblk * r) + 1;
    return LevelGeom{cw, (cw + wpb - 1) / wpb};
}

constexpr u32 NSHARD = 16;
struct StatShard {
    u64 successors;
    u64 enabled;
    u64 probes;
    u64 cas;
    u64 pad[12];
};
struct LevelCounters {
    StatShard stat[NSHARD];
    u32 claims;
    u32 err;
    u32 pad1[30];
    u32 ticket;
    u32 pad2[31];
    u32 gticket[NSHARD][32];
    u32 disc[MAX_PROPS];
    u32 pad3[32];
    u32 prev_claims;
    u32 prev_err;
    u64 next_base;
    u64 unique;
    alignas(128) u32 chunk_next[DYN_SHARDS][32];
    u32 chunk_done;
    u32 pad5[31];
};
static_assert(offsetof(LevelCounters, err) == offsetof(LevelCounters, claims) + 4, "claims/err pair");
static_assert(offsetof(LevelCounters, prev_err) == offsetof(LevelCounters, prev_claims) + 4, "prev pair");
static_assert(offsetof(LevelCounters, claims) % 8 == 0 && offsetof(LevelCounters, prev_claims) % 8 == 0, "u64 loads");

__device__ __forceinline__ void add_stats(LevelCounters* lc, u32 succ, u32 en, u32 probes = 0, u32 cas = 0) {
    StatShard* sh = &lc->stat[blockIdx.x % NSHARD];
    if (succ) atomicAdd(reinterpret_cast<unsigned long long*>(&sh->successors), (unsigned long long)succ);
    if (en) atomicAdd(reinterpret_cast<unsigned long long*>(&sh->enabled), (unsigned long long)en);
    if (probes) atomicAdd(reinterpret_cast<unsigned long long*>(&sh->probes), (unsigned long long)probes);
    if (cas) atomicAdd(reinterpret_cast<unsigned long long*>(&sh->cas), (unsigned long long)cas);
}

__device__ __forceinline__ bool take_ticket(LevelCounters* lc) {
    if (gridDim.x <= 128) return atomicAdd(&lc->ticket, 1u) == gridDim.x - 1;
    const u32 g = blockIdx.x % NSHARD;
    const u32 gsize = (gridDim.x - g + NSHARD - 1) / NSHARD;
    if (atomicAdd(&lc->gticket[g][0], 1u) != gsize - 1) return false;
    return atomicAdd(&lc->ticket, 1u) == min(gridDim.x, NSHARD) - 1;
}

__device__ __forceinline__ u64 gather_stats(const LevelCounters* lc, u32 lane) {
    const u64* w = reinterpret_cast<const u64*>(&lc->stat[lane & (NSHARD - 1)]) + (lane >> 4);
    u64 v = __hip_atomic_load(w, __ATOMIC_RELAXED, __HIP_MEMORY_SCOPE_AGENT);
#pragma unroll
    for (int d = 8; d >= 1; d >>= 1) v += __shfl_xor(v, d, 64);
    return v;
}

__device__ __forceinline__ void reset_stats_tickets(LevelCounters* lc, u32 lane, bool stats) {
    if (stats) reinterpret_cast<u64*>(&lc->stat[lane & (NSHARD - 1)])[lane >> 4] = 0;
// ... 83 lines not shown
    }
    reset_stats_tickets(lc, lane, reset);
    asm volatile("s_waitcnt vmcnt(0)" ::: "memory");
    __builtin_amdgcn_fence(__ATOMIC_RELEASE, "");
    if (lane == 0) __hip_atomic_store(&h->seq, seq, __ATOMIC_RELEASE, __HIP_MEMORY_SCOPE_SYSTEM);
}

template <int = 0> __global__ void publish_kernel(LevelCounters* lc, HostCounters* h, u32 seq, u32 reset, const u32* aux) {
    publish<MAX_PROPS>(lc, h, seq, reset != 0, aux);
}

constexpr u32 SLOTS = 4;
enum SlotFlags : u32 {
    SLOT_REPAIR = 1,
    SLOT_ACTION_TABLE = 2,
};
struct SlotWork {
    const u32* prev_n;
    const LevelCounters* pub;
    HostCounters* hc;
    u32 seq;
    LevelCounters* zero;
    u32 flags = 0;
    const u32* peb = nullptr;
    u32* naeb = nullptr;
    u64 room = 0;
    u32 gmul = 0;
    const LevelCounters* chain = nullptr;
    u64* arena = nullptr;
    u32* apar = nullptr;
    u64 arena_cap = 0;
    u64 fbase = 0;
    u64 ubase = 0;
};

template <int NP>
__device__ __forceinline__ void slot_service(const SlotWork& sw, u32 lane) {
    if (sw.pub) {
        const LevelCounters* lc = sw.pub;
        u32* hw = reinterpret_cast<u32*>(sw.hc);
        const u64 st = gather_stats(lc, lane);
        if ((lane & 15) == 0) {
            hw[(lane >> 4) * 2] = (u32)st;
            hw[(lane >> 4) * 2 + 1] = (u32)(st >> 32);
        }
        const u32* src = lane == 0 ? &lc->claims : lane == 1 ? &lc->err : lane >= 3 && lane < 3 + NP ? &lc->disc[lane - 3] : nullptr;
        const u32 v = src ? __hip_atomic_load(src, __ATOMIC_RELAXED, __HIP_MEMORY_SCOPE_AGENT) : 0u;
        if (lane == 0) sw.hc->claims = v;
        if (lane == 1) sw.hc->err = v;
        if (lane == 2) sw.hc->aux = 0;
        if (lane >= 3 && lane < 3 + NP) sw.hc->disc[lane - 3] = v;
        asm volatile("s_waitcnt vmcnt(0)" ::: "memory");
        __builtin_amdgcn_fence(__ATOMIC_RELEASE, "");
        if (lane == 0) __hip_atomic_store(&sw.hc->seq, sw.seq, __ATOMIC_RELEASE, __HIP_MEMORY_SCOPE_SYSTEM);
    }
    if (sw.zero) {
        LevelCounters* z = sw.zero;
        reinterpret_cast<u64*>(&z->stat[lane & (NSHARD - 1)])[lane >> 4] = 0;
        if (lane == 0) z->claims = 0;
        if (lane == 1) z->err = 0;
        if (lane < MAX_PROPS) z->disc[lane] = ~0u;
    }
}

template <int NP>
__global__ void slot_publish_kernel(SlotWork sw) {
    slot_service<NP>(sw, threadIdx.x);
}

template <int POL, class T>
__device__ __forceinline__ T probe_load(const T* p) {
    if constexpr (POL == 1) return __hip_atomic_load(p, __ATOMIC_RELAXED, __HIP_MEMORY_SCOPE_AGENT);
    else if constexpr (POL == 2) return __builtin_nontemporal_load(p);
    else if constexpr (POL == 3) return __hip_atomic_load(p, __ATOMIC_RELAXED, __HIP_MEMORY_SCOPE_SYSTEM);
    else return *p;
}

template <int POL = 0>
__device__ __forceinline__ u64 find_or_claim_from(const TableView& t, const ProbeKey& k, u64 cur, bool* is_new,
                                                  u32* err, u32* probes = nullptr, u32* cas = nullptr) {
    const u64 step = probe_step(t);
    const int limit = (int)t.plimit;
    u64 i = k.home, key = k.tag;
    for (int probe = 0; probe < limit; ++probe) {
        if (cur == key) {
            *is_new = false;
            return i;
        }
        if (cur == 0) {
            if (cas) ++*cas;
            const u64 prev = slot_cas(t, i, key);
            if (prev == 0) {
                *is_new = true;
                return i;
            }
            if (prev == key) {
                *is_new = false;
                return i;
            }
        }
        i = (i + 1) & t.mask;
        key += step;
        cur = slot_load<POL>(t, i);
        if (probes) ++*probes;
    }
    atomicOr(err, (u32)ERR_TABLE_FULL);
    *is_new = false;
    return ~0ull;
}

__device__ __forceinline__ u64 find_or_claim(const TableView& t, const ProbeKey& k, bool* is_new, u32* err) {
    return find_or_claim_from(t, k, slot_load(t, k.home), is_new, err);
}

__device__ __forceinline__ u64 find_slot(const TableView& t, const ProbeKey& k) {
    const u64 step = probe_step(t);
    u64 i = k.home, key = k.tag;
    for (int probe = 0; probe < MAX_PROBE; ++probe) {
        const u64 cur = slot_load(t, i);
        if (cur == key) return i;
        if (cur == 0) return ~0ull;
        i = (i + 1) & t.mask;
        key += step;
    }
    return ~0ull;
}

template <class M, class F>
__host__ __device__ __forceinline__ void for_each_successor(const M& m, const u64* s, F&& f) {
    u64 mask[M::MW];
    m.enabled(s, mask);
#pragma unroll
    for (int w = 0; w < M::MW; ++w) {
        u64 bits = mask[w];
        while (bits) {
            int a = w * 64 + __builtin_ctzll(bits);
            bits &= bits - 1;
            u64 ns[M::W];
            if (m.apply(s, a, ns)) f(a, ns);
        }
    }
}

template <int W>
__device__ __forceinline__ void load_state(const u64* base, u64 r, u64* s) {
    if constexpr (W == 2) {
        auto v = reinterpret_cast<const ulonglong2*>(base)[r];
        s[0] = v.x;
        s[1] = v.y;
    } else {
#pragma unroll
        for (int i = 0; i < W; ++i) s[i] = base[r * W + i];
    }
}
template <int W>
__device__ __forceinline__ void store_state(u64* base, u64 r, const u64* s) {
    if constexpr (W == 2) {
        reinterpret_cast<ulonglong2*>(base)[r] = make_ulonglong2(s[0], s[1]);
    } else {
#pragma unroll
        for (int i = 0; i < W; ++i) base[r * W + i] = s[i];
    }
}

template <int W>
__device__ __forceinline__ bool same_state(const u64* a, const u64* b) {
    bool eq = true;
#pragma unroll
    for (int i = 0; i < W; ++i) eq &= a[i] == b[i];
    return eq;
}

template <class M>
__global__ void insert_roots(M m, TableView t, const u64* states, u32 n, LevelCounters* lc) {
    u32 r = blockIdx.x * blockDim.x + threadIdx.x;
    if (r >= n) return;
    u64 s[M::W];
    load_state<M::W>(states, r, s);
    bool is_new;
    u64 slot = find_or_claim(t, probe_key(m, t, s), &is_new, &lc->err);
    if (is_new) {
        if (t.meta) t.meta[slot] = 0;
        atomicAdd(&lc->claims, 1u);
    }
}

template <class M>
__device__ __forceinline__ void eval_props(const M& m, const u64* s, u32 rank, u32 undiscovered, LevelCounters* lc) {
    u32 und = undiscovered;
    while (und) {
        int p = __builtin_ctz(und);
        und &= und - 1;
        if (m.discovers(p, s)) atomicMin(&lc->disc[p], rank);
    }
    if constexpr (has_faulted<M>::value) {
        if (m.faulted(s)) atomicOr(&lc->err, (u32)ERR_MODEL);
    }
}

__device__ __forceinline__ void wave_lds_sync() {
    asm volatile("s_waitcnt lgkmcnt(0)" ::: "memory");
    __builtin_amdgcn_wave_barrier();
}

// ... 354 lines not shown
            const u32 excl = incl - cnt;
            for (u32 j0 = w0; j0 < wend; j0 += 64) {
                const u32 j = j0 + (u32)lane;
                u32 p = 0;
#pragma unroll
                for (int q = 1; q < 8; ++q) {
                    const u32 ex = lane_u32(excl, (u32)q);
                    if ((u32)q < ppw && ex <= j) p = (u32)q;
                }
                const u32 k = j - (u32)__shfl((int)excl, (int)p, 64);
                const u64 m0 = __shfl(mk[0], (int)p, 64);
                const u64 m1 = MW > 1 ? __shfl(mk[MW > 1 ? 1 : 0], (int)p, 64) : 0ull;
                const u32 c0 = (u32)__popcll(m0);
                const u32 a = k < c0 ? select_bit(m0, k) : 64u + select_bit(m1, k - c0);
                if (j < wend) smap[wid][j - w0] = (u16)(p | a << 6);
            }
        } else
        while (nidx < wend && nidx < incl) {
            u32 a = 0;
#pragma unroll
            for (int w = MW - 1; w >= 0; --w)
                if (mk[w]) a = (u32)w * 64 + (u32)__builtin_ctzll(mk[w]);
            mk[a >> 6] &= mk[a >> 6] - 1;
            smap[wid][nidx - w0] = (u16)((u32)lane | a << 6);
            ++nidx;
        }
#if SR_TIMELINE
        if (tl_first_chunk) SR_TL(12);
#endif
        wave_lds_sync();
#if SR_TIMELINE
        if (tl_first_chunk) SR_TL(3);
        tl_first_chunk = false;
#endif

        if constexpr (PB < 0) {
            constexpr int R = -PB;
            constexpr bool FP_ONLY = !has_qkey<M>::value;
            for (u32 s0 = w0; s0 < wend; s0 += 64u * R) {
                u64 kh[FP_ONLY ? 1 : R], kt[R];
                u32 vmask = 0;
#pragma unroll
                for (int r = 0; r < R; ++r) {
                    if (!FP_ONLY) kh[FP_ONLY ? 0 : r] = 0;
                    kt[r] = 0;
                    const u32 i = s0 + (u32)r * 64u + (u32)lane;
                    u32 te = 0;
                    u64 tp = 0, tq = 0;
                    if (tbl) {
                        te = i < wend ? smap[wid][i - w0] : 0u;
                        tp = pst[wid][(te & 63) * W];
                        tq = atab.next(tp, te >> 6);
                    }
                    if (i < wend) {
                        u64 ps[W], q[W];
                        bool ok = true;
                        if (tbl) {
                            ps[0] = tp, q[0] = tq;
                        } else {
                            const u32 e = smap[wid][i - w0];
                            const u32 p = e & 63, a = e >> 6;
#pragma unroll
                            for (int x = 0; x < W; ++x) ps[x] = pst[wid][p * W + x];
                            ok = m.apply(ps, (int)a, q);
                        }
                        if (ok) {
                            ++succ;
                            if constexpr (!exact_moves_model<M>) ok = !same_state<W>(q, ps);
                        }
                        if (ok) {
                            const ProbeKey k = probe_key(m, t, q);
                            if (fmask)
                                ok = !filter_seen(filt, fcompact, filt_log2, fmask, t, filter_key(t, k));
                            if (!FP_ONLY) kh[FP_ONLY ? 0 : r] = k.home;
                            kt[r] = k.tag;
                        }
                        if (ok) vmask |= 1u << r;
                    }
                }
#if SR_TIMELINE
                if (tl_first_round) SR_TL(4);
#endif
                u32 nmask = 0;
                u32 st = 0, cr = 0, disp = 0;
                u64 si = 0, tag = 0;
                const u64 step = probe_step(t);
                for (;;) {
                    if (st == 0 && vmask) {
                        cr = (u32)__builtin_ctz(vmask);
                        vmask &= vmask - 1;
                        tag = kt[0];
#pragma unroll
                        for (int r = 1; r < R; ++r)
                            if (cr == (u32)r) tag = kt[r];
                        if constexpr (FP_ONLY) {
                            si = tag & t.mask;
                        } else {
                            si = kh[0];
#pragma unroll
                            for (int r = 1; r < R; ++r)
                                if (cr == (u32)r) si = kh[FP_ONLY ? 0 : r];
                        }
                        st = 1;
                        disp = 0;
                    }
                    if (!__ballot(st != 0)) break;
                    u64 v = 0;
                    if (st == 1) v = slot_load<POL>(t, si);
                    if (st == 2) v = slot_cas(t, si, tag);
                    if constexpr (STATS) {
                        probes += st == 1;
                        cas += st == 2;
                    }
                    if (st != 0) {
                        if (v == tag) {
                            st = 0;
                        } else if (v == 0) {
                            if (st == 2) nmask |= 1u << cr;
                            st = st == 1 ? 2u : 0u;
                        } else if (++disp >= t.plimit) {
                            atomicOr(&lc->err, (u32)ERR_TABLE_FULL);
                            st = 0;
                        } else {
                            si = (si + 1) & t.mask;
                            tag += step;
                            st = 1;
                        }
                    }
                }
#if SR_TIMELINE
                if (tl_first_round) SR_TL(5);
                tl_first_round = false;
#endif
#pragma unroll
                for (int r = 0; r < R; ++r) {
                    const bool nw = nmask >> r & 1;
                    u64 q[W];
                    u32 p = 0;
                    if (tbl) {
                        if (__ballot(nw)) {
                            const u32 e = nw ? smap[wid][s0 + (u32)r * 64u + (u32)lane - w0] : 0u;
                            p = e & 63;
                            q[0] = atab.next(pst[wid][p * W], e >> 6);
                        }
                    } else if (nw) {
                        const u32 e = smap[wid][s0 + (u32)r * 64u + (u32)lane - w0];
                        p = e & 63;
                        u64 ps[W];
#pragma unroll
                        for (int x = 0; x < W; ++x) ps[x] = pst[wid][p * W + x];
                        m.apply(ps, (int)(e >> 6), q);
                    }
                    append_new(nw, q, p);
                }
            }
        } else
        for (u32 it = w0; it < wend; it += 64 * PB) {
            u64 ns[PB][W], cur[PB];
            ProbeKey pk[PB];
            u32 par[PB];
            bool ok[PB];
#pragma unroll
            for (int j = 0; j < PB; ++j) {
                const u32 i = it + j * 64 + lane;
                ok[j] = i < wend;
                par[j] = 0;
                if (tbl) {
                    const u32 e = ok[j] ? smap[wid][i - w0] : 0u;
                    par[j] = e & 63;
                    const u64 ps0 = pst[wid][par[j] * W];
                    ns[j][0] = atab.next(ps0, e >> 6);
                    if constexpr (!exact_moves_model<M>) {
                        if (ok[j] && ns[j][0] == ps0) {
                            ++succ;
                            ok[j] = false;
                        }
                    }
                } else if (ok[j]) {
                    const u32 e = smap[wid][i - w0];
                    const u32 p = e & 63, a = e >> 6;
                    u64 ps[W];
#pragma unroll
                    for (int x = 0; x < W; ++x) ps[x] = pst[wid][p * W + x];
                    ok[j] = m.apply(ps, (int)a, ns[j]);
                    par[j] = p;
                    if constexpr (!exact_moves_model<M>) {
                        if (ok[j] && same_state<W>(ns[j], ps)) {
                            ++succ;
                            ok[j] = false;
                        }
                    }
                }
                pk[j] = ok[j] ? probe_key(m, t, ns[j]) : ProbeKey{0, 0};
                if (fmask && ok[j]) {
                    if (filter_seen(filt, fcompact, filt_log2, fmask, t, filter_key(t, pk[j]))) {
                        ++succ;
                        ok[j] = false;
                    }
                }
            }
#pragma unroll
            for (int j = 0; j < PB; ++j) {
                cur[j] = ok[j] ? slot_load<POL>(t, pk[j].home) : 0;
// ... 287 lines not shown
    u64 s[M::W];
    load_state<M::W>(frontier, r, s);
    u32 und = undiscovered;
    while (und) {
        int p = __builtin_ctz(und);
        und &= und - 1;
        if (m.discovers(p, s)) atomicMin(&lc->disc[p], r);
    }
}

template <class M>
__global__ void __launch_bounds__(256) roots_fused(M m, TableView t, const u64* states, u32 n, LevelCounters* lc,
                                                   u32 undiscovered, HostCounters* h, u32 seq) {
    const u32 r = threadIdx.x;
    if (r < n) {
        u64 s[M::W];
        load_state<M::W>(states, r, s);
        bool is_new;
        const u64 slot = find_or_claim(t, probe_key(m, t, s), &is_new, &lc->err);
        if (is_new) {
            if (t.meta) t.meta[slot] = 0;
            atomicAdd(&lc->claims, 1u);
        }
        for (u32 und = undiscovered; und; und &= und - 1) {
            const int p = __builtin_ctz(und);
            if (m.discovers(p, s)) atomicMin(&lc->disc[p], r);
        }
    }
    publish<M::NPROPS>(lc, h, seq, true, nullptr);
}

__device__ __forceinline__ void init_counter_words(LevelCounters* lc, LevelCounters* slots, u32 nslots) {
    constexpr u32 WORDS = sizeof(LevelCounters) / 4;
    constexpr u32 D0 = offsetof(LevelCounters, disc) / 4;
    for (u32 i = threadIdx.x; i < WORDS * (1 + nslots); i += blockDim.x) {
        const u32 o = i % WORDS;
        u32* w = i < WORDS ? reinterpret_cast<u32*>(lc) + i : reinterpret_cast<u32*>(slots) + (i - WORDS);
        *w = o >= D0 && o < D0 + MAX_PROPS ? ~0u : 0u;
    }
}
template <int = 0> __global__ void init_level_counters(LevelCounters* lc, LevelCounters* slots, u32 nslots) {
    init_counter_words(lc, slots, nslots);
}

constexpr u32 ROOTS_INLINE_WORDS = 32;
struct InlineStates {
    u64 w[ROOTS_INLINE_WORDS];
};
template <class M>
__global__ void __launch_bounds__(256) roots_start(M m, TableView t, InlineStates init, u32 n, u64* arena, u32* apar,
                                                   u32* aeb, u32 emask, LevelCounters* lc, LevelCounters* slots,
                                                   u32 nslots, u32 undiscovered, HostCounters* h, u32 seq) {
    constexpr int W = M::W;
    init_counter_words(lc, slots, nslots);
    for (u32 i = threadIdx.x; i < n * W; i += blockDim.x) arena[i] = init.w[i];
    for (u32 i = threadIdx.x; i < n; i += blockDim.x) {
        apar[i] = ~0u;
        if (aeb) aeb[i] = emask;
    }
    __syncthreads();
    const u32 r = threadIdx.x;
    if (r < n) {
        u64 s[W];
#pragma unroll
        for (int i = 0; i < W; ++i) s[i] = init.w[r * W + i];
        bool is_new;
        const u64 slot = find_or_claim(t, probe_key(m, t, s), &is_new, &lc->err);
        if (is_new) {
            if (t.meta) t.meta[slot] = 0;
            atomicAdd(&lc->claims, 1u);
        }
        for (u32 und = undiscovered; und; und &= und - 1) {
            const int p = __builtin_ctz(und);
            if (m.discovers(p, s)) atomicMin(&lc->disc[p], r);
        }
    }
    publish<M::NPROPS>(lc, h, seq, true, nullptr);
}

template <int = 0> __global__ void rehash(TableView from, u64 from_cap, TableView to, u32* err) {
    u64 i = (u64)blockIdx.x * blockDim.x + threadIdx.x;
    if (i >= from_cap) return;
    const u64 k = slot_load(from, i);
    if (!k) return;
    bool is_new;
    u64 slot = find_or_claim(to, reprobe(from, to, i, k), &is_new, err);
    if (slot == ~0ull) return;
    if (to.meta) to.meta[slot] = from.meta[i];
}

constexpr u32 REBUILD_BLOCK = 256;
constexpr u32 REBUILD_ROWS = 4;
constexpr u32 REBUILD_BYTES = 32768;
template <class T>
constexpr u32 rebuild_slots() { return REBUILD_BYTES / sizeof(T); }
inline bool rehash_by_ranges(const TableView& from, const TableView& to, u32 lg, u64 cap) {
    const u64 S = to.s32 ? rebuild_slots<u32>() : rebuild_slots<u64>();
    return from.qbits && to.qbits && from.qbits == to.qbits + lg && (1ull << lg) <= S && cap % S == 0;
}
template <class T>
__global__ void __launch_bounds__(REBUILD_BLOCK)
    rehash_ranges(TableView from, u64 from_cap, TableView to, u32 lg, u64* spill, u64 spill_cap, u32* err) {
    constexpr u32 S = rebuild_slots<T>();
    __shared__ uint4 lds4[REBUILD_BYTES / 16];
    T* lds = reinterpret_cast<T*>(lds4);
    for (u32 j = threadIdx.x; j < REBUILD_BYTES / 16; j += REBUILD_BLOCK) lds4[j] = make_uint4(0, 0, 0, 0);
    __syncthreads();
    const u64 r0 = (u64)blockIdx.x * S;
    const u64 a = r0 >> lg, span = S >> lg;
    const u64 omask = from_cap - 1, dmask = (1ull << from.dbits) - 1;
    u64 lo = 0, hi = min<u64>(span + REBUILD_BLOCK, from_cap);
    for (;;) {
        bool done = false;
        for (u64 base = lo; base < hi; base += REBUILD_ROWS * REBUILD_BLOCK) {
            u64 v[REBUILD_ROWS];
#pragma unroll
            for (u32 r = 0; r < REBUILD_ROWS; ++r) {
                const u64 off = base + r * REBUILD_BLOCK + threadIdx.x;
                v[r] = off < hi ? slot_load(from, (a + off) & omask) : 1ull;
            }
#pragma unroll
            for (u32 r = 0; r < REBUILD_ROWS; ++r) {
                const u64 off = base + r * REBUILD_BLOCK + threadIdx.x, i = (a + off) & omask;
                if (off >= hi) continue;
                if (!v[r]) {
                    done |= off >= span;
                    continue;
                }
                if (((i - ((v[r] & dmask) - 1) - a) & omask) >= span) continue;
                const ProbeKey k = quot_probe(to, quot_decode(from, i, v[r]));
                u64 j = k.home - r0;
                if (j >= S) {
                    atomicOr(err, (u32)ERR_TABLE_FULL);
                    continue;
                }
                for (u64 d = 0;; ++d, ++j) {
                    if (d >= to.plimit) {
                        atomicOr(err, (u32)ERR_TABLE_FULL);
                        break;
                    }
                    if (j >= S) {
                        const u64 q = atomicAdd(reinterpret_cast<unsigned long long*>(spill), 1ull);
                        if (q < spill_cap) spill[1 + q] = i;
                        else atomicOr(err, (u32)ERR_TABLE_FULL);
                        break;
                    }
                    if (atomicCAS(&lds[j], (T)0, (T)(k.tag + d)) == (T)0) break;
                }
            }
        }
        if (__syncthreads_or(done) || hi >= from_cap) break;
        lo = hi;
        hi = min<u64>(hi + REBUILD_BLOCK, from_cap);
    }
    uint4* out = reinterpret_cast<uint4*>(reinterpret_cast<T*>(to.keys) + r0);
    for (u32 j = threadIdx.x; j < REBUILD_BYTES / 16; j += REBUILD_BLOCK) out[j] = lds4[j];
}
template <int = 0>
__global__ void rehash_spill(TableView from, TableView to, const u64* spill, u64 spill_cap, u32* err) {
    const u64 n = min(spill[0], spill_cap);
    for (u64 q = (u64)blockIdx.x * blockDim.x + threadIdx.x; q < n; q += (u64)gridDim.x * blockDim.x) {
        const u64 i = spill[1 + q];
        bool is_new;
        (void)find_or_claim(to, reprobe(from, to, i, slot_load(from, i)), &is_new, err);
    }
}

template <int = 0> __global__ void __launch_bounds__(256) table_max_disp(TableView t, u64 cap, u32* out) {
    u32 best = 0;
    const u64 dmask = t.qbits ? (1ull << t.dbits) - 1 : 0;
    for (u64 i = (u64)blockIdx.x * blockDim.x + threadIdx.x; i < cap; i += (u64)gridDim.x * blockDim.x) {
        const u64 v = slot_load(t, i);
        if (!v) continue;
        const u64 d = t.qbits ? (v & dmask) - 1 : (i - (v & t.mask)) & t.mask;
        best = max(best, (u32)min<u64>(d, 0xffffffffull));
    }
#pragma unroll
    for (int d = 32; d >= 1; d >>= 1) best = max(best, (u32)__shfl_xor((int)best, d, 64));
    if ((threadIdx.x & 63) == 0 && best) atomicMax(out, best);
}

template <int = 0> __global__ void remap_slots(u32* cand, u64 n, TableView from, TableView to) {
    u64 i = (u64)blockIdx.x * blockDim.x + threadIdx.x;
    if (i >= n) return;
    u32 s = cand[i];
    if (s == CAND_NONE) return;
    cand[i] = (u32)find_slot(to, reprobe(from, to, s, slot_load(from, s)));
}

constexpr int SCAN_BLOCK = 256;
constexpr int SCAN_ITEMS = 8;
constexpr int SCAN_TILE = SCAN_BLOCK * SCAN_ITEMS;

__device__ __forceinline__ u32 block_exclusive_scan(u32 v, u32* total) {
    __shared__ u32 wsum[SCAN_BLOCK / 64];
    const int lane = threadIdx.x & 63, wid = threadIdx.x >> 6;
    const u32 x = wave_incl_scan(v);
    if (lane == 63) wsum[wid] = x;
    __syncthreads();
    u32 base = 0, tot = 0;
#pragma unroll
    for (int w = 0; w < SCAN_BLOCK / 64; ++w) {
        if (w < wid) base += wsum[w];
        tot += wsum[w];
    }
    __syncthreads();
    *total = tot;
    return base + x - v;
}

template <int = 0> __global__ void __launch_bounds__(SCAN_BLOCK) scan_tile_sums(const u32* in, u32 n, u32* sums) {
    u64 base = (u64)blockIdx.x * SCAN_TILE + threadIdx.x * SCAN_ITEMS;
    u32 acc = 0;
#pragma unroll
    for (int i = 0; i < SCAN_ITEMS; ++i)
        if (base + i < n) acc += in[base + i];
    u32 tot;
    block_exclusive_scan(acc, &tot);
    if (threadIdx.x == 0) sums[blockIdx.x] = tot;
}

template <int = 0> __global__ void __launch_bounds__(SCAN_BLOCK) scan_sums(u32* sums, u32 nt, u32* grand_total) {
    u32 carry = 0;
    for (u32 base = 0; base < nt; base += SCAN_BLOCK) {
        u32 i = base + threadIdx.x;
        u32 v = i < nt ? sums[i] : 0;
        u32 tot;
        u32 ex = block_exclusive_scan(v, &tot);
        if (i < nt) sums[i] = ex + carry;
        carry += tot;
        __syncthreads();
    }
    if (threadIdx.x == 0) *grand_total = carry;
}

template <int = 0> __global__ void __launch_bounds__(SCAN_BLOCK) scan_tiles(const u32* in, u32 n, const u32* sums, u32* out) {
    u64 base = (u64)blockIdx.x * SCAN_TILE + threadIdx.x * SCAN_ITEMS;
    u32 v[SCAN_ITEMS];
    u32 acc = 0;
#pragma unroll
    for (int i = 0; i < SCAN_ITEMS; ++i) {
        v[i] = base + i < n ? in[base + i] : 0;
        acc += v[i];
    }
    u32 tot;
    u32 ex = block_exclusive_scan(acc, &tot) + sums[blockIdx.x];
#pragma unroll
    for (int i = 0; i < SCAN_ITEMS; ++i) {
        if (base + i < n) out[base + i] = ex;
        ex += v[i];
    }
}

}
```

stateright_amd/csrc/kernels_dist.hpp:

```cpp
#pragma once
#include "kernels.hpp"

namespace sr {

constexpr int GID_SHIFT = 40;
constexpr u32 SENDC_STRIDE = 32;
constexpr u64 PAR_SEARCH = ~0ull - 1;

__device__ __host__ __forceinline__ u32 owner_of(u64 fp, u32 nparts) { return (u32)(((fp >> 32) * (u64)nparts) >> 32); }
#ifndef SR_OKEY_HASH
#define SR_OKEY_HASH 1
#endif
__device__ __host__ __forceinline__ u32 key_owner(u64 key, u32 nparts) {
#if SR_OKEY_HASH
    const u32 h = (u32)key * 0x9E3779B1u ^ (u32)(key >> 32) * 0x85EBCA77u;
    return (u32)(((u64)h * nparts) >> 32);
#else
    return owner_of(fmix64(key * 0x9E3779B97F4A7C15ull + 0x632BE59BD9B4E019ull), nparts);
#endif
}
template <class M>
__device__ __host__ __forceinline__ u32 part_of(const M& m, const u64* s, u64 fp, u32 nparts) {
    if constexpr (has_owner_key<M>::value) {
        u64 key;
// ... 289 lines not shown
                            const ProbeKey pk = probe_key(m, t, q);
                            const u64 key = route_key(m, t, pk, q);
                            if (fmask) {
                                const u64 old = atomicExch(reinterpret_cast<unsigned long long*>(&filt[filter_index(t, key) & fmask]),
                                                           (unsigned long long)key);
                                ok = old != key;
                            }
                            if (ok) {
                                own = route_owner(m, t, q, key, nparts);
                                rem = self_rec || own != my_part;
                                if (!rem) {
                                    vmask |= 1u << r;
                                    kt[r] = pk.tag;
                                    if (!FP_ONLY) kh[FP_ONLY ? 0 : r] = pk.home;
                                }
                            }
                        }
                    }
                    const u64 rmask = __ballot(rem);
                    if (!rmask) continue;
                    const u32 rcnt = __popcll(rmask);
                    const u32 rbelow = __popcll(rmask & lanes_below);
                    const int rleader = __builtin_ctzll(rmask);
                    u32 rsb = 0;
                    if (lane == rleader) rsb = atomicAdd(&rstage_n, rcnt);
                    rsb = lane_u32(rsb, (u32)rleader);
                    const u32 rin = rsb >= RSTAGE ? 0u : min(rcnt, RSTAGE - rsb);
                    if (rem && rbelow < rin) {
                        const u32 kk = rsb + rbelow;
#pragma unroll
                        for (int x = 0; x < W; ++x) rstage[kk * REC + x] = q[x];
                        rown[kk] = (u8)own;
                    }
                    u64 om = __ballot(rem && rbelow >= rin);
                    if (om && lane == 0) sent_any = 1;
                    while (om) {
                        const int leader = __builtin_ctzll(om);
                        const u32 qo = lane_u32(own, (u32)leader);
                        const bool mine = rem && rbelow >= rin && own == qo;
                        const u64 qm = __ballot(mine);
                        om &= ~qm;
                        u32 gb = 0;
                        if (lane == leader) gb = atomicAdd(&send_counts[qo * SENDC_STRIDE], (u32)__popcll(qm));
                        gb = lane_u32(gb, (u32)leader);
                        if (mine) {
                            const u32 pos = gb + __popcll(qm & lanes_below);
                            if (pos < bucket_cap) {
                                u64* rec = sdst[qo] + (u64)pos * REC;
                                u64 v = 0;
#pragma unroll
                                for (int x = 0; x < W; ++x) rec[x] = q[x], v += q[x];
                                if (my_dsum) atomicAdd(reinterpret_cast<unsigned long long*>(&my_dsum[qo]), (unsigned long long)v);
                            } else {
                                atomicOr(&lc->err, (u32)ERR_FRONTIER_OVERFLOW);
                            }
                        }
                    }
                }
                u32 nmask = 0, st = 0, cr = 0, disp = 0;
                u64 si = 0, tag = 0;
                const u64 step = probe_step(t);
                for (;;) {
                    if (st == 0 && vmask) {
                        cr = (u32)__builtin_ctz(vmask);
                        vmask &= vmask - 1;
                        tag = kt[0];
#pragma unroll
                        for (int r = 1; r < R; ++r)
                            if (cr == (u32)r) tag = kt[r];
                        if constexpr (FP_ONLY) {
                            si = tag & t.mask;
                        } else {
                            si = kh[0];
#pragma unroll
                            for (int r = 1; r < R; ++r)
                                if (cr == (u32)r) si = kh[FP_ONLY ? 0 : r];
                        }
                        st = 1;
                        disp = 0;
                    }
                    if (!__ballot(st != 0)) break;
                    u64 v = 0;
                    if (st == 1) v = slot_load<0>(t, si);
                    if (st == 2) v = slot_cas(t, si, tag);
                    if (st != 0) {
                        if (v == tag) {
                            st = 0;
                        } else if (v == 0) {
                            if (st == 2) nmask |= 1u << cr;
                            st = st == 1 ? 2u : 0u;
                        } else if (++disp >= t.plimit) {
                            atomicOr(&lc->err, (u32)ERR_TABLE_FULL);
                            st = 0;
                        } else {
                            si = (si + 1) & t.mask;
                            tag += step;
                            st = 1;
                        }
                    }
                }
#pragma unroll
                for (int r = 0; r < R; ++r) {
                    const bool nw = nmask >> r & 1;
                    const u64 mask = __ballot(nw);
                    if (!mask) continue;
                    u64 q[W];
                    u32 p = 0;
                    if (nw) {
                        const u32 e = smap[wid][s0 + (u32)r * 64u + (u32)lane - w0];
                        p = e & 63;
                        u64 ps[W];
#pragma unroll
                        for (int x = 0; x < W; ++x) ps[x] = pst[wid][p * W + x];
                        m.apply(ps, (int)(e >> 6), q);
                    }
                    const u32 cnt = __popcll(mask);
                    const u32 below = __popcll(mask & lanes_below);
                    const int leader = __builtin_ctzll(mask);
                    u32 sb = 0;
                    if (lane == leader) sb = atomicAdd(&stage_n, cnt);
                    sb = lane_u32(sb, (u32)leader);
                    const u32 in_stage = sb >= (u32)STAGE ? 0u : min(cnt, (u32)STAGE - sb);
                    u32 gb = 0;
                    if (cnt > in_stage && lane == leader) gb = atomicAdd(&lc->claims, cnt - in_stage);
                    gb = lane_u32(gb, (u32)leader);
                    if (!nw) continue;
                    if (below < in_stage) {
                        const u32 kk = sb + below;
#pragma unroll
                        for (int x = 0; x < W; ++x) stage[kk * W + x] = q[x];
                        stage_par[kk] = (u32)(wave0 + p);
                    } else {
                        const u32 pos = gb + (below - in_stage);
                        if (pos < next_cap) {
                            store_state<W>(next, pos, q);
                            next_par[pos] = gid_base + wave0 + p;
                        } else {
                            atomicOr(&lc->err, (u32)ERR_FRONTIER_OVERFLOW);
                        }
                        eval_props(m, q, pos, undiscovered, lc);
                    }
                }
            }
        } else
        for (u32 it = w0; it < wend; it += 64 * PB) {
            u64 ns[PB][W], key[PB], cur[PB];
            ProbeKey pk[PB];
            u32 par[PB], own[PB];
            bool ok[PB], rem[PB];
#pragma unroll
            for (int j = 0; j < PB; ++j) {
                const u32 i = it + j * 64 + lane;
                ok[j] = i < wend;
                par[j] = 0;
                if (ok[j]) {
                    const u32 e = smap[wid][i - w0];
                    const u32 p = e & 63, a = e >> 6;
                    u64 ps[W];
#pragma unroll
                    for (int x = 0; x < W; ++x) ps[x] = pst[wid][p * W + x];
                    ok[j] = m.apply(ps, (int)a, ns[j]);
                    par[j] = p;
                    if (ok[j] && same_state<W>(ns[j], ps)) {
                        ++succ;
                        ok[j] = false;
                    }
                }
// ... 158 lines not shown
    if (lag)
        for (u32 i = threadIdx.x; i < nparts * rw; i += blockDim.x) {
            const u32 q = i / rw, w = i - q * rw;
            (sdst[q] - DIST_HDR)[w] = srow[w];
        }
    if (dsum && lag)
        for (u32 q = threadIdx.x; q < nparts; q += blockDim.x) {
            u64 rs = 0;
            for (u32 w = 0; w < rw; ++w) rs += srow[w];
            u64* hdr = sdst[q] - DIST_HDR;
            hdr[HDR_SEQ] = fseq;
            hdr[HDR_SUM] = hsum[q] + rs;
        }
    if (threadIdx.x < 64) reset_stats_tickets(lc, threadIdx.x, true);
    if (!ftab) return;
    asm volatile("s_waitcnt vmcnt(0)" ::: "memory");
    __syncthreads();
    if (threadIdx.x == 0) __builtin_amdgcn_fence(__ATOMIC_RELEASE, "");
    __syncthreads();
    for (u32 q = threadIdx.x; q < nparts; q += blockDim.x)
        __hip_atomic_store(ftab[q], fseq, __ATOMIC_RELAXED, __HIP_MEMORY_SCOPE_SYSTEM);
}

template <int IPB, class M, class RecAt>
__device__ __forceinline__ void insert_records(const M& m, RecAt rec_at, u32 total, const TableView& t, u64* next,
                                               u64* next_par, u32 next_cap, LevelCounters* lc, u32 undiscovered,
                                               u64* stage, u32 STAGE, u32& stage_n, u32& base, u64& rsum) {
    constexpr int W = M::W;
    const int lane = threadIdx.x & 63;
    auto flush = [&](u32 nl) {
        if (threadIdx.x == 0) base = atomicAdd(&lc->claims, nl);
        __syncthreads();
        for (u32 k = threadIdx.x; k < nl; k += blockDim.x) {
            const u32 pos = base + k;
            u64 ns[W];
#pragma unroll
            for (int x = 0; x < W; ++x) ns[x] = stage[k * W + x];
            if (pos < next_cap) {
                store_state<W>(next, pos, ns);
                next_par[pos] = PAR_SEARCH;
            } else {
                atomicOr(&lc->err, (u32)ERR_FRONTIER_OVERFLOW);
            }
            eval_props(m, ns, pos, undiscovered, lc);
        }
        __syncthreads();
        if (threadIdx.x == 0) stage_n = 0;
    };
    if constexpr (IPB < 0) {
        constexpr int R = -IPB;
        const u64 per_round = (u64)gridDim.x * blockDim.x * R;
        const u64 step = probe_step(t);
        for (u64 g0 = (u64)blockIdx.x * blockDim.x * R; g0 < total; g0 += per_round) {
            __syncthreads();
            u64 ns[R][W], si[R], tag[R];
            u32 st[R], disp[R];
            bool nws[R];
#pragma unroll
            for (int j = 0; j < R; ++j) {
                const u64 g = g0 + (u64)j * blockDim.x + threadIdx.x;
                st[j] = g < total ? 1u : 0u;
                disp[j] = 0;
                nws[j] = false;
                si[j] = tag[j] = 0;
                if (st[j]) {
                    const u64* rec = rec_at((u32)g);
#pragma unroll
                    for (int x = 0; x < W; ++x) ns[j][x] = rec[x], rsum += rec[x];
                    const ProbeKey pk = probe_key(m, t, ns[j]);
                    si[j] = pk.home;
                    tag[j] = pk.tag;
                }
            }
            for (;;) {
                u32 live = 0;
#pragma unroll
                for (int j = 0; j < R; ++j) live |= st[j];
                if (!__ballot(live != 0)) break;
                u64 v[R];
#pragma unroll
                for (int j = 0; j < R; ++j) {
                    v[j] = 0;
                    if (st[j] == 1) v[j] = slot_load(t, si[j]);
                    if (st[j] == 2) v[j] = slot_cas(t, si[j], tag[j]);
                }
#pragma unroll
                for (int j = 0; j < R; ++j) {
                    if (!st[j]) continue;
                    if (v[j] == tag[j]) {
                        st[j] = 0;
                    } else if (v[j] == 0) {
                        nws[j] = st[j] == 2;
                        st[j] = st[j] == 1 ? 2u : 0u;
                    } else if (++disp[j] >= t.plimit) {
                        atomicOr(&lc->err, (u32)ERR_TABLE_FULL);
                        st[j] = 0;
                    } else {
                        si[j] = (si[j] + 1) & t.mask;
                        tag[j] += step;
                        st[j] = 1;
                    }
                }
            }
#pragma unroll
            for (int j = 0; j < R; ++j) {
                const bool nw = nws[j];
                const u64 mask = __ballot(nw);
                if (!mask) continue;
                const u32 cnt = __popcll(mask), below = __popcll(mask & ((1ull << lane) - 1));
                const int leader = __builtin_ctzll(mask);
                u32 sb = 0;
                if (lane == leader) sb = atomicAdd(&stage_n, cnt);
                sb = lane_u32(sb, (u32)leader);
                const u32 in_stage = sb >= STAGE ? 0u : min(cnt, STAGE - sb);
                u32 gb = 0;
                if (cnt > in_stage && lane == leader) gb = atomicAdd(&lc->claims, cnt - in_stage);
                gb = lane_u32(gb, (u32)leader);
                if (!nw) continue;
                if (below < in_stage) {
#pragma unroll
                    for (int x = 0; x < W; ++x) stage[(sb + below) * W + x] = ns[j][x];
                } else {
                    const u32 pos = gb + (below - in_stage);
                    if (pos < next_cap) {
                        store_state<W>(next, pos, ns[j]);
                        next_par[pos] = PAR_SEARCH;
                    } else {
                        atomicOr(&lc->err, (u32)ERR_FRONTIER_OVERFLOW);
                    }
                    eval_props(m, ns[j], pos, undiscovered, lc);
                }
            }
            __syncthreads();
            const u32 sn = min(stage_n, STAGE);
            if (sn >= STAGE / 2) flush(sn);
        }
        __syncthreads();
        const u32 sn = min(stage_n, STAGE);
        if (sn) flush(sn);
        return;
    }
    constexpr int PBI = IPB < 1 ? 1 : IPB;
    const u64 per_round = (u64)gridDim.x * blockDim.x * PBI;
    for (u64 g0 = (u64)blockIdx.x * blockDim.x * PBI; g0 < total; g0 += per_round) {
        __syncthreads();
        u64 ns[PBI][W], cur[PBI];
        ProbeKey pk[PBI];
        bool ok[PBI];
#pragma unroll
        for (int j = 0; j < PBI; ++j) {
            const u64 g = g0 + (u64)j * blockDim.x + threadIdx.x;
            ok[j] = g < total;
            pk[j] = ProbeKey{0, 0};
            if (ok[j]) {
                const u64* rec = rec_at((u32)g);
#pragma unroll
                for (int x = 0; x < W; ++x) ns[j][x] = rec[x], rsum += rec[x];
                pk[j] = probe_key(m, t, ns[j]);
            }
        }
#pragma unroll
        for (int j = 0; j < PBI; ++j) cur[j] = ok[j] ? slot_load(t, pk[j].home) : 0;
        bool nws[PBI];
#pragma unroll
        for (int j = 0; j < PBI; ++j) {
            nws[j] = false;
            if (ok[j] && cur[j] != pk[j].tag) find_or_claim_from(t, pk[j], cur[j], &nws[j], &lc->err);
// ... 288 lines not shown
```

stateright_amd/csrc/table_selftest.hpp:

```cpp
#pragma once
#include <algorithm>
#include <string>
#include <vector>

#include "kernels.hpp"

namespace sr {

struct TableEncoding {
    u32 qbits, dbits, bbits, plimit, s32;
    u32 filter;
    u32 filter_log2;
    u32 min_cap_log2;
};
template <int W>
inline TableEncoding table_encoding_of(int B, u64 cap) {
    const Spread<W> m{B, 1, 0, 0};
    const TableView v = make_table_view(m, nullptr, nullptr, cap, true);
    TableEncoding e{v.qbits, v.dbits, v.bbits, v.plimit, v.s32, 0, 0, 0};
    u32 fl = filter_exact(m) ? default_filter_log2<W>() : 0;
    e.filter = fl ? 1 : 0;
    if (fl && filter_compact_ok(m, fl + 1)) fl += 1, e.filter = 2;
    e.filter_log2 = fl;
    while ((1ull << e.min_cap_log2) < min_table_cap(m)) ++e.min_cap_log2;
// ... 62 lines not shown
                return why = "slot fields do not fill the slot" + where(cap), false;
            if (t.plimit != encoding_probe_limit(t.qbits, t.dbits) || t.plimit < 1)
                return why = "probe limit differs from the encoding's" + where(cap), false;
        } else if (t.s32 || t.plimit != (u32)MAX_PROBE) {
            return why = "fingerprint mode with narrow slots or a short probe limit" + where(cap), false;
        }
        pairs.clear();
        std::vector<std::pair<u64, u64>> fkeys;
        for (const Sample& s : keys) {
            const ProbeKey pk = probe_key(m, t, s.w);
            if (pk.home > t.mask) return why = "home slot past the table" + where(cap), false;
            const u64 step = probe_step(t);
            for (u64 d : {(u64)0, (u64)t.plimit - 1}) {
                const u64 v = pk.tag + d * step;
                if (!v) return why = "a slot value of 0 (vacant)" + where(cap), false;
                if (t.s32 && v >> 32) return why = "slot value does not fit 32 bits" + where(cap), false;
                if (t.qbits) {
                    const u128 h = quot_hash(m, t, s.w);
                    if (B < 128 && h >> B) return why = "permuted key past 2^B" + where(cap), false;
                    if (quot_decode(t, (pk.home + d) & t.mask, v) != h)
                        return why = "slot value at displacement " + std::to_string(d) + " does not decode to the permuted key " +
                                     u128_text(h) + where(cap), false;
                } else if (v != state_fp<Spread<W>>(s.w) || pk.home != (v & t.mask)) {
                    return why = "fingerprint slot is not the state's fingerprint" + where(cap), false;
                }
            }
            pairs.emplace_back(pk.home, pk.tag);
            const u64 fk = filter_key(t, pk);
            fkeys.emplace_back(fk, 0);
            if (fexact && t.qbits && (u128)fk != quot_hash(m, t, s.w) + 1)
                return why = "filter key is not the permuted key + 1" + where(cap), false;
            if (fexact && !fk) return why = "filter key 0 (the empty entry)" + where(cap), false;
            const u32 fl = default_filter_log2<W>() + 1;
            if (filter_compact_ok(m, fl) && (!t.qbits || (fk >> fl) >> 31))
                return why = "compact filter entry loses bits of the filter key" + where(cap), false;
        }
        if ((t.qbits || W == 1) && has_duplicate(pairs)) return why = "two keys share home and slot value" + where(cap), false;
        if (fexact && has_duplicate(fkeys)) return why = "filter key is not injective" + where(cap), false;
        for (u32 lg : {1u, 3u, 6u}) {
            const u64 cap2 = cap << lg;
            if (cap2 > (1ull << MAX_LOG2)) continue;
            const TableView to = make_table_view(m, nullptr, nullptr, cap2, true);
            auto at = [&]() { return where(cap) + " -> 2^" + std::to_string(__builtin_ctzll(cap2)); };
            if ((t.qbits != 0) != (to.qbits != 0))
                return why = std::string("growth switches the mode from ") + (t.qbits ? "quotient to fingerprint" : "fingerprint to quotient") +
                             at(), false;
            const bool ranges = rehash_by_ranges(t, to, lg, cap2);
            if (ranges) {
                const u64 S = to.s32 ? rebuild_slots<u32>() : rebuild_slots<u64>();
                if ((S >> lg) == 0 || cap2 % S || (cap2 / S) >> 32) return why = "rehash_ranges' ranges do not tile the table" + at(), false;
            }
            for (const Sample& s : keys) {
                const ProbeKey pf = probe_key(m, t, s.w), want = probe_key(m, to, s.w);
                for (u64 d : {(u64)0, std::min<u64>(t.plimit - 1, 5)}) {
                    const ProbeKey got = reprobe(t, to, (pf.home + d) & t.mask, pf.tag + d * probe_step(t));
                    if (got.home != want.home || got.tag != want.tag)
                        return why = "reprobe gives home " + std::to_string(got.home) + " value " + std::to_string(got.tag) +
                                     ", probe_key " + std::to_string(want.home) + " / " + std::to_string(want.tag) + at(), false;
                }
                if (ranges && (want.home >> lg) != pf.home) return why = "rehash by ranges, but new home >> lg is not the old home" + at(), false;
            }
        }
    }
    return true;
}

template <int W>
bool check_words(std::string& why) {
    for (int B = 2; B <= std::min(64 * W, 128); ++B) {
        if (W == 4 && B != 18 && B != 24 && B != 50 && B != 60 && B != 78 && B != 79 && B != 96 && B != 97 && B != 120 && B != 128) continue;
        const Spread<W> m{B, 1, 0, 0};
        if (min_table_cap(m) > (1ull << MAX_LOG2)) continue;
        if (!check_model<W>(B, why)) return false;
    }
    return true;
}

}

inline bool table_growth_selftest(std::string& why) {
    return growth_test::check_words<1>(why) && growth_test::check_words<2>(why) && growth_test::check_words<4>(why);
}

}
```

Baseline: 7.035 billion unique states/s.

## Recycle hash tables across runs with epoch-tagged slots instead of memset clears

Adds epoch bits to each hash-table slot so that a recycled table from the pool can be reused by advancing the epoch, rather than being zeroed with a full-table memset on release and reuse. Slots whose epoch field differs from the current epoch read as vacant, and CAS now compares against the observed stale value instead of zero. This is meant to remove the HBM cost of clearing large tables between runs. In exchange it spends key bits on the epoch, which adds complexity to the probe, decode and rehash paths. Only tables above a minimum byte size get epochs, and a clear is forced when the epoch would wrap.

```diff
diff --git a/include/stateright_gpu.h b/include/stateright_gpu.h
--- a/include/stateright_gpu.h
+++ b/include/stateright_gpu.h
@@ -80,6 +80,8 @@
     uint32_t owner_key;
     uint32_t balanced_levels;
     uint32_t table_encoding;
+    uint32_t table_epoch;
+    uint32_t table_clears;
 } sr_stats;
 
 typedef struct sr_bfs sr_bfs;
@@ -166,6 +168,8 @@
 int32_t sr_selftest_action_masks(void);
 int32_t sr_selftest_table_growth(void);
 int32_t sr_table_encoding(int32_t words, int32_t key_bits, uint64_t slots, uint32_t* out);
+int32_t sr_selftest_table_epochs(void);
+int32_t sr_table_epoch_bits(int32_t words, int32_t key_bits, uint64_t slots, int32_t want, uint32_t* out);
 sr_bfs* sr_gpu_bfs_spawn_partitioned(sr_dist* comm, int32_t virtual_partitions, int32_t model_id,
                                      const int64_t* params, int32_t nparams, const sr_opts* opts);
 
diff --git a/stateright_amd/_native.py b/stateright_amd/_native.py
--- a/stateright_amd/_native.py
+++ b/stateright_amd/_native.py
@@ -64,6 +64,8 @@
         ("owner_key", ctypes.c_uint32),
         ("balanced_levels", ctypes.c_uint32),
         ("table_encoding", ctypes.c_uint32),
+        ("table_epoch", ctypes.c_uint32),
+        ("table_clears", ctypes.c_uint32),
     ]
 
     def as_dict(self):
@@ -164,6 +166,9 @@
     ("sr_selftest_models", ctypes.c_int32, []),
     ("sr_selftest_action_masks", ctypes.c_int32, []),
     ("sr_selftest_table_growth", ctypes.c_int32, []),
+    ("sr_selftest_table_epochs", ctypes.c_int32, []),
+    ("sr_table_epoch_bits", ctypes.c_int32, [ctypes.c_int32, ctypes.c_int32, ctypes.c_uint64, ctypes.c_int32,
+                                             ctypes.POINTER(ctypes.c_uint32)]),
     ("sr_table_encoding", ctypes.c_int32, [ctypes.c_int32, ctypes.c_int32, ctypes.c_uint64, ctypes.POINTER(ctypes.c_uint32)]),
     ("sr_gpu_bfs_spawn_plugin", _P, [_P, _I64P, ctypes.c_int32, ctypes.POINTER(sr_opts)]),
     ("sr_gpu_bfs_spawn_plugin_partitioned", _P, [_P, _P, ctypes.c_int32, _I64P, ctypes.c_int32,
@@ -235,6 +240,14 @@
     return dict(zip(("qbits", "dbits", "bbits", "plimit", "s32", "filter", "filter_log2", "min_cap_log2"), out))
 
 
+def table_epoch_bits(words, key_bits, slots, want=-1):
+    out = (ctypes.c_uint32 * 4)()
+    st = load().sr_table_epoch_bits(words, key_bits, slots, want, out)
+    if st != 0:
+        raise ValueError(f"sr_table_epoch_bits: {last_error()} (status {st})")
+    return dict(zip(("ebits", "dbits", "plimit", "last_epoch"), out))
+
+
 def runtime_versions():
     lib = load()
     out = {}
diff --git a/stateright_amd/csrc/device.hpp b/stateright_amd/csrc/device.hpp
--- a/stateright_amd/csrc/device.hpp
+++ b/stateright_amd/csrc/device.hpp
@@ -73,6 +73,11 @@
     const hipError_t e = hipStreamCreateWithFlags(s, hipStreamNonBlocking);
     if (e == hipSuccess) StreamCensus::get().created(dev);
     return e;
+}
+
+inline uint32_t next_epoch_of(uint32_t blk_epoch, uint32_t blk_enc, uint32_t enc, uint32_t last_epoch) {
+    if (blk_epoch == 0) return 1;
+    return enc && blk_enc == enc && blk_epoch < last_epoch ? blk_epoch + 1 : 0;
 }
 
 class DevicePool {
@@ -119,23 +124,31 @@
         std::lock_guard<std::mutex> g(mu_);
         free_[{dev, round(bytes), kind}].push_back(p);
     }
-    void free_zeroed(int dev, void* p, size_t bytes, hipEvent_t ready, int kind = 0) {
-        std::lock_guard<std::mutex> g(mu_);
-        zeroed_[{dev, round(bytes), kind}].push_back({p, ready});
-    }
-    void* alloc_zeroed(int dev, size_t bytes, hipStream_t s, int kind = 0) {
-        Zeroed z{nullptr, nullptr};
+    void free_zeroed(int dev, void* p, size_t bytes, hipEvent_t ready, int kind = 0, uint32_t epoch = 0, uint32_t enc = 0) {
+        std::lock_guard<std::mutex> g(mu_);
+        zeroed_[{dev, round(bytes), kind}].push_back({p, ready, epoch, enc});
+    }
+    void* alloc_zeroed(int dev, size_t bytes, hipStream_t s, int kind = 0, uint32_t enc = 0, uint32_t last_epoch = 0,
+                       uint32_t* epoch = nullptr, bool* dirty = nullptr) {
+        Zeroed z{nullptr, nullptr, 0, 0};
+        if (epoch) *epoch = 1;
+        if (dirty) *dirty = false;
         {
             std::lock_guard<std::mutex> g(mu_);
             auto& fl = zeroed_[{dev, round(bytes), kind}];
             if (fl.empty()) return nullptr;
-            size_t pick = 0;
-            for (size_t i = 0; i < fl.size(); ++i)
-                if (hipEventQuery(fl[i].ready) == hipSuccess) {
-                    pick = i;
-                    break;
-                }
+            auto clean = [&](const Zeroed& c) { return next_epoch_of(c.epoch, c.enc, enc, last_epoch) != 0; };
+            size_t pick = fl.size();
+            int best = -1;
+            for (size_t i = 0; i < fl.size(); ++i) {
+                if (!clean(fl[i]) && !dirty) continue;
+                const int score = (!clean(fl[i]) ? 0 : fl[i].epoch ? 4 : 2) + (hipEventQuery(fl[i].ready) == hipSuccess ? 1 : 0);
+                if (score > best) best = score, pick = i;
+            }
             clear_not_ready();
+            if (pick == fl.size()) return nullptr;
+            if (!clean(fl[pick])) *dirty = true;
+            else if (epoch) *epoch = next_epoch_of(fl[pick].epoch, fl[pick].enc, enc, last_epoch);
             z = fl[pick];
             fl.erase(fl.begin() + (long)pick);
         }
@@ -188,6 +201,8 @@
     struct Zeroed {
         void* p;
         hipEvent_t ready;
+        uint32_t epoch;
+        uint32_t enc;
     };
     void* take_zeroed_locked(int dev, size_t bytes) {
         auto it = zeroed_.find({dev, bytes, 0});
@@ -234,22 +249,29 @@
         kind = k;
         p = static_cast<T*>(DevicePool::get().alloc(d, n * sizeof(T), k));
     }
-    void alloc_zero(int d, size_t count, hipStream_t s, int k = 0) {
+    void alloc_zero(int d, size_t count, hipStream_t s, int k = 0) { (void)alloc_epoch(d, count, s, k, 0, 0); }
+    uint32_t alloc_epoch(int d, size_t count, hipStream_t s, int k, uint32_t enc, uint32_t last_epoch, bool* cleared = nullptr) {
         reset();
         dev = d;
         n = count ? count : 1;
         kind = k;
-        p = static_cast<T*>(DevicePool::get().alloc_zeroed(d, n * sizeof(T), s, k));
-        if (p) return;
-        p = static_cast<T*>(DevicePool::get().alloc(d, n * sizeof(T), k));
-        SR_HIP(hipMemsetAsync(p, 0, n * sizeof(T), s));
-    }
-    void release_zero(hipStream_t s) noexcept {
+        uint32_t epoch = 1;
+        bool dirty = false;
+        p = static_cast<T*>(DevicePool::get().alloc_zeroed(d, n * sizeof(T), s, k, enc, last_epoch, &epoch, &dirty));
+        if (!p) {
+            p = static_cast<T*>(DevicePool::get().alloc(d, n * sizeof(T), k));
+            dirty = true;
+        }
+        if (dirty) SR_HIP(hipMemsetAsync(p, 0, n * sizeof(T), s));
+        if (cleared) *cleared = dirty;
+        return dirty ? 1u : epoch;
+    }
+    void release_zero(hipStream_t s, uint32_t epoch = 0, uint32_t enc = 0) noexcept {
         if (!p) return;
         hipEvent_t ready = nullptr;
         if (hipEventCreateWithFlags(&ready, hipEventDisableTiming) == hipSuccess) {
-            if (hipMemsetAsync(p, 0, n * sizeof(T), s) == hipSuccess && hipEventRecord(ready, s) == hipSuccess) {
-                DevicePool::get().free_zeroed(dev, p, n * sizeof(T), ready, kind);
+            if ((epoch || hipMemsetAsync(p, 0, n * sizeof(T), s) == hipSuccess) && hipEventRecord(ready, s) == hipSuccess) {
+                DevicePool::get().free_zeroed(dev, p, n * sizeof(T), ready, kind, epoch, enc);
                 p = nullptr;
                 n = 0;
                 kind = 0;
diff --git a/stateright_amd/csrc/engine.hip b/stateright_amd/csrc/engine.hip
--- a/stateright_amd/csrc/engine.hip
+++ b/stateright_amd/csrc/engine.hip
@@ -918,6 +918,40 @@
             return SR_ERR_ARG;
         }
         return SR_OK;
+    } catch (const std::exception& x) {
+        set_error(x.what());
+        return SR_ERR_ARG;
+    }
+}
+
+int32_t sr_selftest_table_epochs(void) {
+    try {
+        std::string why;
+        if (!table_epoch_selftest(why)) {
+            set_error(why);
+            return SR_ERR_ARG;
+        }
+        return SR_OK;
+    } catch (const std::exception& x) {
+        set_error(x.what());
+        return SR_ERR_ARG;
+    }
+}
+
+int32_t sr_table_epoch_bits(int32_t words, int32_t key_bits, uint64_t slots, int32_t want, uint32_t* out) {
+    try {
+        if (!out || key_bits < 2 || (words != 1 && words != 2 && words != 4) || key_bits > std::min(64 * words, 128) ||
+            !slots || (slots & (slots - 1)) || want < -1)
+            throw Error(SR_ERR_ARG, "sr_table_epoch_bits: words 1, 2 or 4, 2 <= key_bits <= min(64 words, 128), slots a power of two, want >= -1");
+        auto view = [&](auto m) { return make_table_view(m, nullptr, nullptr, slots, true, want < 0 ? epoch_bits_env() : want, 1); };
+        const TableView v = words == 1 ? view(Spread<1>{key_bits, 1, 0, 0}) : words == 2 ? view(Spread<2>{key_bits, 1, 0, 0})
+                                                                                         : view(Spread<4>{key_bits, 1, 0, 0});
+        const u32 o[4] = {v.ebits, v.dbits, v.plimit, last_epoch(v.ebits)};
+        std::copy(o, o + 4, out);
+        return SR_OK;
+    } catch (const Error& x) {
+        set_error(x.what());
+        return x.code;
     } catch (const std::exception& x) {
         set_error(x.what());
         return SR_ERR_ARG;
diff --git a/stateright_amd/csrc/engine.hpp b/stateright_amd/csrc/engine.hpp
--- a/stateright_amd/csrc/engine.hpp
+++ b/stateright_amd/csrc/engine.hpp
@@ -285,6 +285,7 @@
         if (const char* e = std::getenv("SR_CHAIN_MAX")) chain_max_ = (u64)std::max(0ll, std::atoll(e));
         if (const char* e = std::getenv("SR_TABLE_KIND")) table_kind_ = std::atoi(e);
         if (const char* e = std::getenv("SR_TABLE_RECYCLE")) table_recycle_ = std::atoi(e) != 0;
+        epoch_env_ = epoch_bits_env();
         if (const char* e = std::getenv("SR_BALANCE")) balance_ = std::atoi(e) != 0;
         if (const char* e = std::getenv("SR_BALANCE_MIN")) balance_min_ = (u64)std::max(0ll, std::atoll(e));
         action_table_ = action_table_model<M> && A_ <= 64;
@@ -435,15 +436,27 @@
     }
 
   private:
-    TableView view() const { return make_table_view(m_, keys_.p, fifo_ ? meta_.p : nullptr, cap_); }
+    TableView view() const { return view_of(keys_.p, fifo_ ? meta_.p : nullptr, cap_, epoch_); }
+    int epoch_want() const { return table_recycle_ && !fifo_ && !o_.counters ? epoch_env_ : 0; }
+    TableView view_of(u64* keys, u64* meta, u64 cap, u32 epoch, bool natural = false) const {
+        return make_table_view(m_, keys, meta, cap, natural, epoch_want(), epoch);
+    }
+    static u32 table_enc(const TableView& v) { return v.ebits ? v.ebits | v.dbits << 8 | (v.s32 ? 1u << 16 : 0u) : 0u; }
 
     void alloc_table(u64 cap, bool zero = true) {
         cap_ = cap;
         lmax_ = max_load(cap);
-        const u64 words = table_words(make_table_view(m_, nullptr, nullptr, cap), cap);
+        const TableView v0 = view_of(nullptr, nullptr, cap, 0);
+        const u64 words = table_words(v0, cap);
         table_unzeroed_ = false;
-        if (zero) keys_.alloc_zero(o_.device, words, stream_, table_kind_);
-        else keys_.alloc(o_.device, words, table_kind_);
+        epoch_ = 1;
+        if (zero) {
+            bool cleared = false;
+            epoch_ = keys_.alloc_epoch(o_.device, words, stream_, table_kind_, table_enc(v0), last_epoch(v0.ebits), &cleared);
+            stats.table_clears += cleared;
+        } else {
+            keys_.alloc(o_.device, words, table_kind_);
+        }
         if (fifo_) {
             meta_.alloc(o_.device, cap);
             SR_HIP(hipMemsetAsync(meta_.p, 0xff, cap * sizeof(u64), stream_));
@@ -456,7 +469,7 @@
         DBuf<u64> ok, om;
         ok.swap(keys_);
         if (fifo_) om.swap(meta_);
-        const TableView from = make_table_view(m_, ok.p, fifo_ ? om.p : nullptr, cap_);
+        const TableView from = view_of(ok.p, fifo_ ? om.p : nullptr, cap_, epoch_);
         const u64 old_cap = cap_;
         if (!aux_.p) aux_.alloc(o_.device, 2);
         u64 f0 = 2;
@@ -484,7 +497,7 @@
         check_async_growth_pending_first();
         retired_keys_.emplace_back();
         retired_keys_.back().swap(keys_);
-        const TableView from = make_table_view(m_, retired_keys_.back().p, nullptr, cap_);
+        const TableView from = view_of(retired_keys_.back().p, nullptr, cap_, epoch_);
         const u64 old_cap = cap_;
         if (!aux_.p) aux_.alloc(o_.device, 2);
         u64 f = 2;
@@ -498,7 +511,7 @@
     }
     void launch_rehash(const TableView& from, u64 old_cap, u64 f) {
         const u64 cap = old_cap * f;
-        const TableView to0 = make_table_view(m_, nullptr, nullptr, cap);
+        const TableView to0 = view_of(nullptr, nullptr, cap, 0);
         u32 lg = 0;
         while ((1ull << lg) < f) ++lg;
         const u64 S = to0.s32 ? rebuild_slots<u32>() : rebuild_slots<u64>();
@@ -558,7 +571,7 @@
     u64 grow_first_ = std::getenv("SR_GROW_FIRST") ? (u64)std::atoi(std::getenv("SR_GROW_FIRST")) : 0u;
 
     double max_load(u64 cap) const {
-        const TableView v = make_table_view(m_, nullptr, nullptr, cap, true);
+        const TableView v = view_of(nullptr, nullptr, cap, 0, true);
         return max_load_for(v.plimit, (double)cap, 0.8);
     }
 
@@ -566,6 +579,7 @@
         const TableView v = view();
         stats.displacement_limit = v.plimit;
         stats.table_encoding = table_encoding_word(v, filt_log2_, filt_compact_);
+        stats.table_epoch = v.epoch;
         if (!o_.counters || !cap_) return;
         if (!aux_.p) aux_.alloc(o_.device, 2);
         SR_HIP(hipMemsetAsync(aux_.p + 1, 0, sizeof(u32), stream_));
@@ -1083,7 +1097,10 @@
     }
 
     void release_table() {
-        if (table_recycle_ && !fifo_ && !o_.counters && !table_unzeroed_) keys_.release_zero(stream_);
+        if (!table_recycle_ || fifo_ || o_.counters || table_unzeroed_ || !keys_.p) return;
+        const TableView v = view();
+        if (!v.ebits) stats.table_clears++;
+        keys_.release_zero(stream_, v.ebits ? v.epoch : 0u, table_enc(v));
     }
     void free_unzeroed_table() {
         if (!table_recycle_ || fifo_ || o_.counters || !table_unzeroed_ || !keys_.p) return;
@@ -1347,6 +1364,8 @@
     double queue_ratio_ = std::getenv("SR_QUEUE_RATIO") ? std::atof(std::getenv("SR_QUEUE_RATIO")) : 0.0;
     int ppw_env_ = -1;
     bool table_recycle_ = true;
+    int epoch_env_ = EPOCH_AUTO;
+    u32 epoch_ = 0;
     u32 grid_res_ = 2;
     u32 grid_max_[5] = {0, 0, 0, 0, 0};
     u32 grid_env_ = 0;
diff --git a/stateright_amd/csrc/kernels.hpp b/stateright_amd/csrc/kernels.hpp
--- a/stateright_amd/csrc/kernels.hpp
+++ b/stateright_amd/csrc/kernels.hpp
@@ -55,7 +55,13 @@
     u32 bbits = 0;
     u32 plimit = MAX_PROBE;
     u32 s32 = 0;
+    u32 ebits = 0;
+    u32 epoch = 0;
+    u32 emask = 0;
+    u32 efield = 0;
 };
+
+SR_HD bool slot_vacant(const TableView& t, u64 v) { return v == 0 || ((u32)v & t.emask) != t.efield; }
 
 template <int POL, class T>
 __device__ __forceinline__ T probe_load(const T* p);
@@ -64,9 +70,9 @@
     if (t.s32) return (u64)probe_load<POL>(reinterpret_cast<const u32*>(t.keys) + i);
     return probe_load<POL>(t.keys + i);
 }
-__device__ __forceinline__ u64 slot_cas(const TableView& t, u64 i, u64 tag) {
-    if (t.s32) return (u64)atomicCAS(reinterpret_cast<u32*>(t.keys) + i, 0u, (u32)tag);
-    return atomicCAS(reinterpret_cast<unsigned long long*>(t.keys + i), 0ull, (unsigned long long)tag);
+__device__ __forceinline__ u64 slot_cas(const TableView& t, u64 i, u64 cur, u64 tag) {
+    if (t.s32) return (u64)atomicCAS(reinterpret_cast<u32*>(t.keys) + i, (u32)cur, (u32)tag);
+    return atomicCAS(reinterpret_cast<unsigned long long*>(t.keys + i), (unsigned long long)cur, (unsigned long long)tag);
 }
 SR_HD u64 table_words(const TableView& t, u64 cap) { return t.s32 ? (cap + 1) / 2 : cap; }
 
@@ -122,11 +128,12 @@
 SR_HD u64 probe_step(const TableView& t) { return t.qbits ? 1ull : 0ull; }
 SR_HD ProbeKey fp_probe(const TableView& t, u64 fp) { return ProbeKey{fp & t.mask, fp}; }
 SR_HD ProbeKey quot_probe(const TableView& t, u128 h) {
-    return ProbeKey{(u64)(h >> t.qbits), (((u64)h & ((1ull << t.qbits) - 1)) << t.dbits) | 1ull};
+    return ProbeKey{(u64)(h >> t.qbits),
+                    (((u64)h & ((1ull << t.qbits) - 1)) << (t.dbits + t.ebits)) | (u64)(t.efield | 1u)};
 }
 SR_HD u128 quot_decode(const TableView& t, u64 i, u64 v) {
     const u64 d = (v & ((1ull << t.dbits) - 1)) - 1;
-    return ((u128)((i - d) & t.mask) << t.qbits) | (v >> t.dbits);
+    return ((u128)((i - d) & t.mask) << t.qbits) | (v >> (t.dbits + t.ebits));
 }
 SR_HD ProbeKey reprobe(const TableView& from, const TableView& to, u64 i, u64 v) {
     return from.qbits ? quot_probe(to, quot_decode(from, i, v)) : fp_probe(to, v);
@@ -152,8 +159,27 @@
     (void)m;
     return false;
 }
-template <class M>
-inline TableView make_table_view(const M& m, u64* keys, u64* meta, u64 cap, bool natural = false) {
+constexpr u32 SLOT64_DMIN = 17, SLOT64_DMAX = 24;
+constexpr u32 EPOCH_BITS_MAX = 8;
+constexpr int EPOCH_AUTO = -1;
+constexpr u64 EPOCH_MIN_BYTES = 1ull << 30;
+inline int epoch_bits_env() {
+    const char* e = std::getenv("SR_EPOCH_BITS");
+    return e ? std::max(0, std::min((int)EPOCH_BITS_MAX, std::atoi(e))) : EPOCH_AUTO;
+}
+inline u32 choose_epoch_bits(u32 qbits, bool s32, u64 cap, int want) {
+    if (!qbits || want == 0) return 0;
+    if (want == EPOCH_AUTO && cap * (s32 ? 4 : 8) < EPOCH_MIN_BYTES) return 0;
+    const u32 width = s32 ? 32 : 64, dmin = s32 ? SLOT32_DMIN : SLOT64_DMIN;
+    const u32 spare = width - qbits > dmin ? width - qbits - dmin : 0;
+    if (spare < 2) return 0;
+    return std::min(spare, want == EPOCH_AUTO ? EPOCH_BITS_MAX : (u32)want);
+}
+inline u32 last_epoch(u32 ebits) { return (1u << ebits) - 1; }
+
+template <class M>
+inline TableView make_table_view(const M& m, u64* keys, u64* meta, u64 cap, bool natural = false, int epoch_bits = 0,
+                                 u32 epoch = 0) {
     TableView v{keys, meta, cap - 1};
     if constexpr (has_qkey<M>::value) {
         const u32 B = (u32)m.qkey_bits();
@@ -170,6 +196,13 @@
             } else {
                 v.dbits = 64 - v.qbits;
             }
+            v.ebits = choose_epoch_bits(v.qbits, v.s32 != 0, cap, meta ? 0 : epoch_bits);
+            if (v.ebits) {
+                v.dbits = std::min(v.dbits - v.ebits, v.s32 ? 32u : SLOT64_DMAX);
+                v.epoch = std::max(1u, std::min(epoch, last_epoch(v.ebits)));
+                v.emask = last_epoch(v.ebits) << v.dbits;
+                v.efield = v.epoch << v.dbits;
+            }
         }
     }
     v.plimit = encoding_probe_limit(v.qbits, v.dbits);
@@ -201,7 +234,7 @@
 }
 
 SR_HD u64 filter_key(const TableView& t, const ProbeKey& k) {
-    return t.qbits ? ((k.home << t.qbits) | (k.tag >> t.dbits)) + 1 : k.tag;
+    return t.qbits ? ((k.home << t.qbits) | (k.tag >> (t.dbits + t.ebits))) + 1 : k.tag;
 }
 SR_HD u32 filter_index(const TableView& t, u64 fk) { return t.qbits ? (u32)fk : (u32)(fk >> 40); }
 template <class M>
@@ -218,7 +251,7 @@
     return v.qbits && v.bbits <= 30 + log2_entries;
 }
 inline u32 table_encoding_word(const TableView& t, u32 filt_log2, bool compact) {
-    return t.qbits | (t.s32 ? 1u << 8 : 0u) | filt_log2 << 16 | (compact ? 1u << 24 : 0u);
+    return t.qbits | (t.s32 ? 1u << 8 : 0u) | t.ebits << 12 | filt_log2 << 16 | (compact ? 1u << 24 : 0u);
 }
 __device__ __forceinline__ bool filter_seen(u64* filt, bool compact, u32 flog, u32 fmask, const TableView& t, u64 fk) {
     if (compact) {
@@ -468,27 +501,26 @@
     const u64 step = probe_step(t);
     const int limit = (int)t.plimit;
     u64 i = k.home, key = k.tag;
-    for (int probe = 0; probe < limit; ++probe) {
+    for (int probe = 0; probe < limit;) {
         if (cur == key) {
             *is_new = false;
             return i;
         }
-        if (cur == 0) {
+        if (slot_vacant(t, cur)) {
             if (cas) ++*cas;
-            const u64 prev = slot_cas(t, i, key);
-            if (prev == 0) {
+            const u64 prev = slot_cas(t, i, cur, key);
+            if (prev == cur) {
                 *is_new = true;
                 return i;
             }
-            if (prev == key) {
-                *is_new = false;
-                return i;
-            }
+            cur = prev;
+            continue;
         }
         i = (i + 1) & t.mask;
         key += step;
         cur = slot_load<POL>(t, i);
         if (probes) ++*probes;
+        ++probe;
     }
     atomicOr(err, (u32)ERR_TABLE_FULL);
     *is_new = false;
@@ -505,7 +537,7 @@
     for (int probe = 0; probe < MAX_PROBE; ++probe) {
         const u64 cur = slot_load(t, i);
         if (cur == key) return i;
-        if (cur == 0) return ~0ull;
+        if (slot_vacant(t, cur)) return ~0ull;
         i = (i + 1) & t.mask;
         key += step;
     }
@@ -1026,9 +1058,10 @@
                 if (tl_first_round) SR_TL(4);
 #endif
                 u32 nmask = 0;
-                u32 st = 0, cr = 0, disp = 0;
-                u64 si = 0, tag = 0;
+                u32 st = 0, cr = 0;
+                u64 si = 0, tag = 0, seen = 0;
                 const u64 step = probe_step(t);
+                const u32 dmask = t.dbits >= 32 ? ~0u : (1u << t.dbits) - 1;
                 for (;;) {
                     if (st == 0 && vmask) {
                         cr = (u32)__builtin_ctz(vmask);
@@ -1046,12 +1079,11 @@
                                 if (cr == (u32)r) si = kh[FP_ONLY ? 0 : r];
                         }
                         st = 1;
-                        disp = 0;
                     }
                     if (!__ballot(st != 0)) break;
                     u64 v = 0;
                     if (st == 1) v = slot_load<POL>(t, si);
-                    if (st == 2) v = slot_cas(t, si, tag);
+                    if (st == 2) v = slot_cas(t, si, seen, tag);
                     if constexpr (STATS) {
                         probes += st == 1;
                         cas += st == 2;
@@ -1059,10 +1091,12 @@
                     if (st != 0) {
                         if (v == tag) {
                             st = 0;
-                        } else if (v == 0) {
-                            if (st == 2) nmask |= 1u << cr;
-                            st = st == 1 ? 2u : 0u;
-                        } else if (++disp >= t.plimit) {
+                        } else if (slot_vacant(t, v)) {
+                            const bool won = st == 2 && v == seen;
+                            if (won) nmask |= 1u << cr;
+                            seen = v;
+                            st = won ? 0u : 2u;
+                        } else if ((t.qbits ? (u32)tag & dmask : (u32)((si - tag) & t.mask) + 1) >= t.plimit) {
                             atomicOr(&lc->err, (u32)ERR_TABLE_FULL);
                             st = 0;
                         } else {
@@ -1516,7 +1550,7 @@
     u64 i = (u64)blockIdx.x * blockDim.x + threadIdx.x;
     if (i >= from_cap) return;
     const u64 k = slot_load(from, i);
-    if (!k) return;
+    if (slot_vacant(from, k)) return;
     bool is_new;
     u64 slot = find_or_claim(to, reprobe(from, to, i, k), &is_new, err);
     if (slot == ~0ull) return;
@@ -1557,7 +1591,7 @@
             for (u32 r = 0; r < REBUILD_ROWS; ++r) {
                 const u64 off = base + r * REBUILD_BLOCK + threadIdx.x, i = (a + off) & omask;
                 if (off >= hi) continue;
-                if (!v[r]) {
+                if (slot_vacant(from, v[r])) {
                     done |= off >= span;
                     continue;
                 }
@@ -1605,7 +1639,7 @@
     const u64 dmask = t.qbits ? (1ull << t.dbits) - 1 : 0;
     for (u64 i = (u64)blockIdx.x * blockDim.x + threadIdx.x; i < cap; i += (u64)gridDim.x * blockDim.x) {
         const u64 v = slot_load(t, i);
-        if (!v) continue;
+        if (slot_vacant(t, v)) continue;
         const u64 d = t.qbits ? (v & dmask) - 1 : (i - (v & t.mask)) & t.mask;
         best = max(best, (u32)min<u64>(d, 0xffffffffull));
     }
diff --git a/stateright_amd/csrc/kernels_dist.hpp b/stateright_amd/csrc/kernels_dist.hpp
--- a/stateright_amd/csrc/kernels_dist.hpp
+++ b/stateright_amd/csrc/kernels_dist.hpp
@@ -395,7 +395,7 @@
                     if (!__ballot(st != 0)) break;
                     u64 v = 0;
                     if (st == 1) v = slot_load<0>(t, si);
-                    if (st == 2) v = slot_cas(t, si, tag);
+                    if (st == 2) v = slot_cas(t, si, 0, tag);
                     if (st != 0) {
                         if (v == tag) {
                             st = 0;
@@ -720,7 +720,7 @@
                 for (int j = 0; j < R; ++j) {
                     v[j] = 0;
                     if (st[j] == 1) v[j] = slot_load(t, si[j]);
-                    if (st[j] == 2) v[j] = slot_cas(t, si[j], tag[j]);
+                    if (st[j] == 2) v[j] = slot_cas(t, si[j], 0, tag[j]);
                 }
 #pragma unroll
                 for (int j = 0; j < R; ++j) {
diff --git a/stateright_amd/csrc/table_selftest.hpp b/stateright_amd/csrc/table_selftest.hpp
--- a/stateright_amd/csrc/table_selftest.hpp
+++ b/stateright_amd/csrc/table_selftest.hpp
@@ -168,4 +168,287 @@
     return growth_test::check_words<1>(why) && growth_test::check_words<2>(why) && growth_test::check_words<4>(why);
 }
 
-}
+namespace epoch_test {
+
+struct HostTable {
+    TableView t;
+    std::vector<u64> s;
+};
+
+inline u64 host_find_or_claim(HostTable& h, const ProbeKey& k, bool* is_new) {
+    u64 i = k.home, key = k.tag;
+    for (u32 probe = 0; probe < h.t.plimit; ++probe) {
+        const u64 cur = h.s[i];
+        if (cur == key) return *is_new = false, i;
+        if (slot_vacant(h.t, cur)) return h.s[i] = key, *is_new = true, i;
+        i = (i + 1) & h.t.mask;
+        key += probe_step(h.t);
+    }
+    *is_new = false;
+    return ~0ull;
+}
+inline u64 host_find(const HostTable& h, const ProbeKey& k) {
+    u64 i = k.home, key = k.tag;
+    for (int probe = 0; probe < MAX_PROBE; ++probe) {
+        if (h.s[i] == key) return i;
+        if (slot_vacant(h.t, h.s[i])) return ~0ull;
+        i = (i + 1) & h.t.mask;
+        key += probe_step(h.t);
+    }
+    return ~0ull;
+}
+inline bool host_rehash(const HostTable& from, HostTable& to) {
+    for (u64 i = 0; i <= from.t.mask; ++i) {
+        if (slot_vacant(from.t, from.s[i])) continue;
+        bool nw;
+        if (host_find_or_claim(to, reprobe(from.t, to.t, i, from.s[i]), &nw) == ~0ull || !nw) return false;
+    }
+    return true;
+}
+inline bool host_rehash_ranges(const HostTable& from, HostTable& to, u32 lg, u64 S) {
+    const u64 from_cap = from.t.mask + 1, cap = to.t.mask + 1, dmask = (1ull << from.t.dbits) - 1;
+    std::vector<u64> spill, lds(S);
+    for (u64 r0 = 0; r0 < cap; r0 += S) {
+        std::fill(lds.begin(), lds.end(), 0);
+        const u64 a = r0 >> lg, span = S >> lg;
+        for (u64 off = 0; off < from_cap; ++off) {
+            const u64 i = (a + off) & from.t.mask, v = from.s[i];
+            if (slot_vacant(from.t, v)) {
+                if (off >= span) break;
+                continue;
+            }
+            if (((i - ((v & dmask) - 1) - a) & from.t.mask) >= span) continue;
+            const ProbeKey k = quot_probe(to.t, quot_decode(from.t, i, v));
+            u64 j = k.home - r0;
+            if (j >= S) return false;
+            for (u64 d = 0;; ++d, ++j) {
+                if (d >= to.t.plimit) return false;
+                if (j >= S) {
+                    spill.push_back(i);
+                    break;
+                }
+                if (lds[j] == 0) {
+                    lds[j] = k.tag + d;
+                    break;
+                }
+            }
+        }
+        std::copy(lds.begin(), lds.end(), to.s.begin() + (long)r0);
+    }
+    for (u64 i : spill) {
+        bool nw;
+        if (host_find_or_claim(to, reprobe(from.t, to.t, i, from.s[i]), &nw) == ~0ull || !nw) return false;
+    }
+    return true;
+}
+inline u64 host_occupied(const HostTable& h, u64* max_disp = nullptr) {
+    u64 n = 0, best = 0;
+    const u64 dmask = h.t.qbits ? (1ull << h.t.dbits) - 1 : 0;
+    for (u64 i = 0; i <= h.t.mask; ++i) {
+        const u64 v = h.s[i];
+        if (slot_vacant(h.t, v)) continue;
+        ++n;
+        best = std::max(best, h.t.qbits ? (v & dmask) - 1 : (i - (v & h.t.mask)) & h.t.mask);
+    }
+    if (max_disp) *max_disp = best;
+    return n;
+}
+
+template <class M>
+inline u64 planned_cap(const M& m, u64 unique, int want) {
+    const double load = unique > (1ull << 31) ? 0.75 : 0.3;
+    u64 cap = std::max<u64>(1ull << 22, min_table_cap(m));
+    for (;; cap <<= 1) {
+        const TableView v = make_table_view(m, nullptr, nullptr, cap, true, want);
+        if ((double)cap * std::min(load, max_load_for(v.plimit, (double)cap, 0.8)) >= (double)unique) return cap;
+    }
+}
+
+template <int W>
+bool check_view(int B, u64 cap, int want, double unique, std::string& why) {
+    const Spread<W> m{B, 1, 0, 0};
+    const TableView t0 = make_table_view(m, nullptr, nullptr, cap, true, 0);
+    auto where = [&]() {
+        return " at W=" + std::to_string(W) + " B=" + std::to_string(B) + " cap=2^" + std::to_string(__builtin_ctzll(cap)) +
+               " want=" + std::to_string(want);
+    };
+    const TableView t1 = make_table_view(m, nullptr, nullptr, cap, true, want, 1);
+    const u32 width = t1.s32 ? 32 : 64;
+    if (t1.qbits != t0.qbits || t1.s32 != t0.s32 || t1.bbits != t0.bbits) return why = "epoch bits change the slot width or the remainder" + where(), false;
+    if (!t1.qbits && t1.ebits) return why = "a fingerprint table with epoch bits" + where(), false;
+    if (want == 0 && (t1.ebits || t1.epoch || t1.dbits != t0.dbits || t1.plimit != t0.plimit)) return why = "ebits = 0 differs from the encoding without epochs" + where(), false;
+    if (t1.ebits) {
+        const u32 dmin = t1.s32 ? SLOT32_DMIN : SLOT64_DMIN;
+        if (t1.ebits < (want == 1 ? 1u : 2u) || t1.ebits > EPOCH_BITS_MAX || (want > 0 && t1.ebits > (u32)want)) return why = "epoch width outside the rule" + where(), false;
+        if (t1.dbits < dmin || t1.qbits + t1.ebits + t1.dbits > width || t1.dbits + t1.ebits > 32) return why = "slot fields do not fit the slot" + where(), false;
+        if (!t1.s32 && t1.plimit != (u32)MAX_PROBE) return why = "an 8-byte slot's probe limit moved" + where(), false;
+    } else if (t1.epoch || t1.dbits != t0.dbits) {
+        return why = "no epoch bits, but the view differs" + where(), false;
+    }
+    if (t1.plimit != encoding_probe_limit(t1.qbits, t1.dbits)) return why = "probe limit differs from the narrower field's" + where(), false;
+    if (unique > 0 && t1.plimit < (u32)MAX_PROBE && expected_max_displacement(unique / (double)cap, (double)cap) >= t1.plimit / 2.0)
+        return why = "the planned load's expected longest run reaches half the probe limit" + where(), false;
+    if (unique > 0 && unique / (double)cap > max_load_for(t1.plimit, (double)cap, 0.8)) return why = "the planned load is past max_load_for" + where(), false;
+    u64 r = 0x9E3779B97F4A7C15ull * (u64)(B + 131 * W) + cap;
+    for (int n = 0; n < 48; ++n) {
+        r = fmix64(r + 0x9E3779B97F4A7C15ull);
+        const u128 top = B >= 128 ? ~(u128)0 : ((u128)1 << B) - 1;
+        const u128 key = n == 0 ? 0 : n == 1 ? top : ((((u128)fmix64(r ^ 0xABCDEFull)) << 64) | r) & top;
+        const u64 s[4] = {(u64)key, W >= 2 ? (u64)(key >> 64) : 0, 0, 0};
+        for (u32 e : {1u, last_epoch(t1.ebits)}) {
+            if (!t1.ebits && e != 1) continue;
+            const TableView t = make_table_view(m, nullptr, nullptr, cap, true, want, e);
+            if (t.ebits && t.epoch != e) return why = "the view does not carry the epoch asked for" + where(), false;
+            const ProbeKey pk = probe_key(m, t, s), p0 = probe_key(m, t0, s);
+            if (pk.home != p0.home) return why = "epoch bits move a key's home" + where(), false;
+            if (filter_key(t, pk) != filter_key(t0, p0)) return why = "epoch bits change the filter key" + where(), false;
+            for (u64 d : {(u64)0, (u64)t.plimit - 1}) {
+                const u64 v = pk.tag + d * probe_step(t);
+                if (t.s32 && v >> 32) return why = "slot value does not fit 32 bits" + where(), false;
+                if (slot_vacant(t, v)) return why = "an entry reads vacant at its own epoch" + where(), false;
+                if (t.qbits && quot_decode(t, (pk.home + d) & t.mask, v) != quot_hash(m, t, s)) return why = "slot value does not decode to the permuted key" + where(), false;
+                if (t.qbits && ((v & ((1ull << t.dbits) - 1)) - 1) != d) return why = "displacement field does not hold the displacement" + where(), false;
+                if (!t.ebits) continue;
+                for (u32 o = 1; o <= last_epoch(t.ebits); ++o) {
+                    const TableView u = make_table_view(m, nullptr, nullptr, cap, true, want, o);
+                    if (slot_vacant(u, v) != (o != e)) return why = "a slot of epoch " + std::to_string(e) + " at epoch " + std::to_string(o) + where(), false;
+                    if (quot_decode(u, (pk.home + d) & t.mask, v) != quot_hash(m, t, s)) return why = "decoding depends on the epoch" + where(), false;
+                }
+            }
+        }
+        const TableView any = make_table_view(m, nullptr, nullptr, cap, true, want, 1 + (u32)(r % std::max(1u, last_epoch(t1.ebits))));
+        if (!slot_vacant(any, 0)) return why = "an all-zero slot is not vacant" + where(), false;
+    }
+    return true;
+}
+
+template <int W>
+bool walk(int B, u32 k, int want, u32 lg, std::string& why) {
+    const Spread<W> m{B, 1, 0, 0};
+    const u64 cap = 1ull << k, cap2 = cap << lg;
+    auto where = [&]() { return " (walk W=" + std::to_string(W) + " B=" + std::to_string(B) + " cap=2^" + std::to_string(k) + " want=" + std::to_string(want) + ")"; };
+    auto state = [&](u64 n, u64 salt, u64* s) {
+        const u128 top = ((u128)1 << B) - 1;
+        const u64 a = fmix64(n * 0x9E3779B97F4A7C15ull + salt), b = fmix64(a ^ salt);
+        const u128 key = (((((u128)b << 64) | a) & top) & ~(u128)3) | (u128)(salt & 3);
+        s[0] = (u64)key, s[1] = W >= 2 ? (u64)(key >> 64) : 0, s[2] = s[3] = 0;
+    };
+    HostTable h{make_table_view(m, nullptr, nullptr, cap, true, want, 1), std::vector<u64>(cap, 0)};
+    if (want && !h.t.ebits) return why = "the walk's table has no epoch bits" + where(), false;
+    const u64 nkeys = cap / 2;
+    u64 distinct1 = 0;
+    for (u64 n = 0; n < nkeys; ++n) {
+        u64 s[4];
+        state(n, 1, s);
+        bool nw;
+        if (host_find_or_claim(h, probe_key(m, h.t, s), &nw) == ~0ull) return why = "epoch 1: probe limit reached" + where(), false;
+        distinct1 += nw;
+    }
+    if (host_occupied(h) != distinct1) return why = "epoch 1: occupied slots differ from the claims" + where(), false;
+    if (h.t.ebits) {
+        if (next_epoch_of(1, 7, 7, last_epoch(h.t.ebits)) != 2) return why = "the pool does not advance the epoch" + where(), false;
+        h.t = make_table_view(m, nullptr, nullptr, cap, true, want, 2);
+    } else {
+        std::fill(h.s.begin(), h.s.end(), 0);
+    }
+    if (host_occupied(h) != 0) return why = "epoch 2: the table left full by epoch 1 is not vacant" + where(), false;
+    for (u64 n = 0; n < nkeys; n += 7) {
+        u64 s[4];
+        state(n, 1, s);
+        if (host_find(h, probe_key(m, h.t, s)) != ~0ull) return why = "epoch 2: a key of epoch 1 is found" + where(), false;
+    }
+    u64 distinct2 = 0;
+    std::vector<std::pair<u64, u64>> slots2;
+    for (u64 n = 0; n < nkeys; ++n) {
+        u64 s[4];
+        state(n, n & 1 ? 1 : 2, s);
+        bool nw;
+        const u64 slot = host_find_or_claim(h, probe_key(m, h.t, s), &nw);
+        if (slot == ~0ull) return why = "epoch 2: probe limit reached" + where(), false;
+        distinct2 += nw;
+        if (host_find(h, probe_key(m, h.t, s)) != slot) return why = "epoch 2: lookup does not find the claimed slot" + where(), false;
+    }
+    u64 md = 0;
+    if (host_occupied(h, &md) != distinct2 || md >= h.t.plimit) return why = "epoch 2: occupied slots differ from the claims" + where(), false;
+    for (u64 i = 0; i < cap; ++i) {
+        if (slot_vacant(h.t, h.s[i]) || !h.t.qbits) continue;
+        const u64 d = (h.s[i] & ((1ull << h.t.dbits) - 1)) - 1;
+        for (u64 x = 1; x <= d; ++x)
+            if (slot_vacant(h.t, h.s[(i - x) & h.t.mask])) return why = "epoch 2: a vacant slot between an entry and its home" + where(), false;
+    }
+    for (int ranges = 0; ranges < 2; ++ranges) {
+        HostTable to{make_table_view(m, nullptr, nullptr, cap2, true, want, ranges ? 1 : 2), std::vector<u64>(cap2, 0)};
+        const u64 S = to.t.s32 ? rebuild_slots<u32>() : rebuild_slots<u64>();
+        if (ranges && !rehash_by_ranges(h.t, to.t, lg, cap2)) {
+            if (h.t.qbits && (u32)B > k + lg) return why = "the walk's growth is not one by ranges" + where(), false;
+            continue;
+        }
+        if (ranges) {
+            for (u64 i = 0; i < cap2; ++i) to.s[i] = fmix64(i + 99) >> (to.t.s32 ? 32 : 0);
+            if (!host_rehash_ranges(h, to, lg, S)) return why = "growth by ranges failed" + where(), false;
+        } else {
+            if (to.t.ebits) {
+                const TableView old = make_table_view(m, nullptr, nullptr, cap2, true, want, 1);
+                for (u64 n = 0; n < cap2 / 2; ++n) {
+                    u64 s[4];
+                    state(n, 3, s);
+                    const ProbeKey pk = probe_key(m, old, s);
+                    to.s[pk.home] = pk.tag;
+                }
+            }
+            if (!host_rehash(h, to)) return why = "growth by CAS failed" + where(), false;
+        }
+        if (host_occupied(to) != distinct2) return why = std::string("after growth ") + (ranges ? "by ranges" : "by CAS") + ": occupied slots differ" + where(), false;
+        for (u64 n = 0; n < nkeys; ++n) {
+            u64 s[4];
+            state(n, n & 1 ? 1 : 2, s);
+            if (host_find(to, probe_key(m, to.t, s)) == ~0ull) return why = std::string("after growth ") + (ranges ? "by ranges" : "by CAS") + ": a key is lost" + where(), false;
+            state(n, 3, s);
+            if (!ranges && to.t.ebits && host_find(to, probe_key(m, to.t, s)) != ~0ull) return why = "after growth: a stale key is found" + where(), false;
+        }
+    }
+    return true;
+}
+
+inline bool run(std::string& why) {
+    if (next_epoch_of(0, 0, 5, 3) != 1 || next_epoch_of(0, 0, 0, 0) != 1) return why = "a zeroed block must serve at epoch 1", false;
+    if (next_epoch_of(1, 5, 5, 3) != 2 || next_epoch_of(2, 5, 5, 3) != 3) return why = "a stamped block must serve at its next epoch", false;
+    if (next_epoch_of(3, 5, 5, 3) != 0) return why = "an epoch about to wrap must force a clear", false;
+    if (next_epoch_of(1, 5, 6, 3) != 0 || next_epoch_of(1, 5, 0, 0) != 0) return why = "another encoding must force a clear", false;
+    for (int N = 9; N <= 12; ++N) {
+        const double two_pc = std::pow(6.0, N) + std::pow(4.0, N) + std::pow(2.0, N);
+        double il = 0, term = 1;
+        for (int kk = 1; kk <= N; ++kk) term *= (double)(N - kk + 1), il += term;
+        il = 1 + 4 * il;
+        for (int want = EPOCH_AUTO; want <= (int)EPOCH_BITS_MAX; ++want) {
+            {
+                const Spread<1> m{4 * N + 4, 1, 0, 0};
+                const u64 cap = planned_cap(m, (u64)two_pc, want);
+                if (cap != planned_cap(m, (u64)two_pc, 0)) return why = "epoch bits change 2pc's planned table at N=" + std::to_string(N), false;
+                for (u64 c : {cap / 2, cap, cap * 2})
+                    if (!check_view<1>(4 * N + 4, c, want, c == cap ? two_pc : 0, why)) return false;
+            }
+            {
+                const int B = 5 + 6 * N;
+                const Spread<2> m{B, 1, 0, 0};
+                const u64 cap = planned_cap(m, (u64)il, want);
+                if (cap != planned_cap(m, (u64)il, 0)) return why = "epoch bits change increment_lock's planned table at N=" + std::to_string(N), false;
+                for (u64 c : {cap / 2, cap, cap * 2})
+                    if (c >= min_table_cap(m) && !check_view<2>(B, c, want, c == cap ? il : 0, why)) return false;
+            }
+        }
+    }
+    if (!check_view<1>(64, 1ull << 22, 2, 0, why) || !check_view<2>(120, 1ull << 28, EPOCH_AUTO, 0, why)) return false;
+    for (int want : {2, 0}) {
+        if (!walk<1>(30, 14, want, 1, why) || !walk<1>(44, 13, want, 3, why) || !walk<2>(50, 13, want, 1, why) ||
+            !walk<1>(12, 14, want, 1, why))
+            return false;
+    }
+    return walk<1>(64, 13, 0, 1, why);
+}
+
+}
+
+inline bool table_epoch_selftest(std::string& why) { return epoch_test::run(why); }
+
+}
```

Result: slower. 6.901 billion unique states/s (-1.9%).
